# katehai/m-cedm

Hardware: AMD Instinct MI355X
Metric: denoised_states_per_sec_18step_edm_heun (higher is better)
Workload: dtype f32; 1 GPU; SWE-periodic 128x128, EDM U-Net ch=128 ch_mult=[1,1,1,1] attn@16^2 (BASELINE config 3); states_per_gpu=32, global_batch=32, H=128, W=128, sampler=EDM Heun, 18 steps, 35 NFE/state, S_churn=0, w=0, fp64 state / fp32 net, parallelism=batch-sharded x1, no data-path collective, launch=one HIP graph per sampler call

## Files before the change

### m-cedm_amd/csrc/conv_wino.hip

```cpp
#include <atomic>
#include <cstdlib>

#include "conv_wino.hpp"
#include "pack.hpp"
#include "prof.hpp"

namespace mcedm {

__global__ void wino_pack_kernel(const float* __restrict__ w, float* __restrict__ dst, int Cout, int Cin, int coutp, int nch,
                                 int tflip) {
  const int idx = blockIdx.x * blockDim.x + threadIdx.x;
  if (idx >= coutp * nch * WKC) return;
  wino_pack_elem(w, dst, idx, Cout, Cin, coutp, tflip);
}

__global__ void conv_frag_pack_kernel(const float* __restrict__ w, float* __restrict__ dst, int Cout, int Cin, int coutp, int cinp) {
  const int idx = blockIdx.x * blockDim.x + threadIdx.x;
  if (idx >= coutp * cinp) return;
  dst[idx] = frag_pack_value(w, idx, Cout, Cin, coutp);
}

template <class C, bool = C::SKIP>
struct SkipFold {};
template <class C>
struct SkipFold<C, true> {
  static constexpr int SKS = C::SKS, SKBUF = C::SKBUF, SKP = C::SKPITCH;
  __amdgpu_buffer_rsrc_t rs_a, rs_b;
  unsigned voff, HW4;
  int Ca, nsk;
  const f32x4* wf;
  size_t wstride;
  float* wr;
  const float* rd;
  f32x4 sld, sa[2];

  __device__ __forceinline__ f32x4 req(int s) const {
    const int ci0 = SKS * s;
    if (ci0 < Ca) return __builtin_bit_cast(f32x4, __builtin_amdgcn_raw_buffer_load_b128(rs_a, voff, (unsigned)ci0 * HW4, 0));
    return __builtin_bit_cast(f32x4, __builtin_amdgcn_raw_buffer_load_b128(rs_b, voff, (unsigned)(ci0 - Ca) * HW4, 0));
  }
  __device__ __forceinline__ void commit(int buf) const {
    float* d = wr + buf * SKBUF;
    *reinterpret_cast<f32x2*>(d) = f32x2{sld[0], sld[1]};
    *reinterpret_cast<f32x2*>(d + SKP) = f32x2{sld[2], sld[3]};
  }
  __device__ __forceinline__ void wreq(int s, f32x4 (&a)[2]) const {
    a[0] = wf[(size_t)(2 * s) * wstride];
    a[1] = wf[(size_t)(2 * s + 1) * wstride];
  }
  __device__ __forceinline__ void begin(const ConvArgs& p, float* skbuf, int n, int mblk, int mblocks, int y0, int x0, int tid, int lane, int hf) {
    asm volatile("" : "+v"(tid));
    lane = tid & 63;
    const unsigned HW = (unsigned)p.H * (unsigned)p.W;
    HW4 = 4u * HW;
    Ca = p.sk_Ca;
    nsk = (p.sk_Ca + p.sk_Cb) / SKS;
    rs_a = make_rsrc(p.sk_xa + (size_t)n * p.sk_Ca * HW, 4u * (unsigned)p.sk_Ca * HW);
    rs_b = make_rsrc(p.sk_xb ? p.sk_xb + (size_t)n * p.sk_Cb * HW : nullptr, p.sk_xb ? 4u * (unsigned)p.sk_Cb * HW : 0u);
    const int c16 = tid >> 5, row = (tid & 31) >> 2, q = tid & 3;
    voff = 4u * ((unsigned)c16 * HW + (unsigned)(y0 + row) * (unsigned)p.W + (unsigned)(x0 + 4 * q));
    wr = skbuf + ((row & 1) * 32 + (row >> 1) * WTX + 2 * q) * SKP + (c16 & 1) * 16 + 2 * (c16 >> 1);
    rd = skbuf + (hf * 32 + (lane & 31)) * SKP + (lane >> 5) * 16;
    wf = reinterpret_cast<const f32x4*>(p.sk_wfrag) + (size_t)mblk * 64 + lane;
    wstride = (size_t)mblocks * 64;
    sld = req(0);
    wreq(0, sa);
  }
  __device__ __forceinline__ void run(float* xch, const float* skb, int wave, int pw, int lane, const f32x16 (&keep)[2], const f32x16 (&send)[2],
                                      float (&v0)[16], float (&v1)[16]) {
#pragma unroll
    for (int r = 0; r < 16; ++r) xch[(wave * 16 + r) * 64 + lane] = send[0][r];
    commit(0);
    sld = req(1);
    f32x16 rv[2];
    {
      const f32x16 zero16 = {0.f, 0.f, 0.f, 0.f, 0.f, 0.f, 0.f, 0.f, 0.f, 0.f, 0.f, 0.f, 0.f, 0.f, 0.f, 0.f};
      float z = 0.f;
#pragma unroll
      for (int e = 0; e < 2; ++e) {
        asm volatile("" : "+v"(z));
        rv[e] = __builtin_amdgcn_mfma_f32_32x32x2f32(z, z, zero16, 0, 0, 0);
      }
    }
    __syncthreads();
#pragma unroll
    for (int r = 0; r < 16; ++r) v0[r] = keep[0][r] + xch[(pw * 16 + r) * 64 + lane];
    f32x4 bq[4];
#pragma unroll
    for (int jj = 0; jj < 4; ++jj) bq[jj] = *reinterpret_cast<const f32x4*>(rd + 4 * jj);
    for (int s = 0; s < nsk; ++s) {
      f32x4 bqn[4], san[2];
      wreq(s + 1 < nsk ? s + 1 : s, san);
      commit((s + 1) & 1);
      sld = req(s + 2 < nsk ? s + 2 : nsk - 1);
#pragma unroll
      for (int j = 0; j < 4; ++j)
#pragma unroll
        for (int e = 0; e < 2; ++e) rv[e] = __builtin_amdgcn_mfma_f32_32x32x2f32(sa[j >> 2][j & 3], bq[j >> 1][2 * (j & 1) + e], rv[e], 0, 0, 0);
      __syncthreads();
      const float* b = rd + ((s + 1) & 1) * SKBUF;
#pragma unroll
      for (int jj = 0; jj < 4; ++jj) bqn[jj] = *reinterpret_cast<const f32x4*>(b + 4 * jj);
      if (s == 0) {
#pragma unroll
        for (int r = 0; r < 16; ++r) xch[(wave * 16 + r) * 64 + lane] = send[1][r];
      }
      if (s == 1) {
#pragma unroll
        for (int r = 0; r < 16; ++r) v1[r] = keep[1][r] + xch[(pw * 16 + r) * 64 + lane];
      }
#pragma unroll
      for (int j = 4; j < 8; ++j)
#pragma unroll
        for (int e = 0; e < 2; ++e) rv[e] = __builtin_amdgcn_mfma_f32_32x32x2f32(sa[j >> 2][j & 3], bq[j >> 1][2 * (j & 1) + e], rv[e], 0, 0, 0);
#pragma unroll
      for (int jj = 0; jj < 4; ++jj) bq[jj] = bqn[jj];
      sa[0] = san[0];
      sa[1] = san[1];
    }
#pragma unroll
    for (int r = 0; r < 16; ++r) {
      const float bs = skb[(r & 3) + 8 * (r >> 2)];
      v0[r] = v0[r] + (rv[0][r] + bs);
      v1[r] = v1[r] + (rv[1][r] + bs);
    }
  }
};

template <class C, bool UP, bool ACT = true, class... Tag>
__global__ __launch_bounds__(C::NT, C::MB == 4 ? 1 : 2) void conv_wino_kernel(const ConvArgs p, int tiles_x, int tiles_img, int nch, int mblocks,
                                                                          int per, int mode) {
  constexpr int WSC = C::SC, VBUF = C::VBUF, RBUF = C::RBUF, MB = C::MB;
  constexpr bool SKIP = C::SKIP;
  constexpr bool UPZ = WinoUpTraits<Tag...>::UPZ;
  constexpr bool UPS = WinoUpTraits<Tag...>::UPS;
  static_assert(!UPS || UPZ, "source-resolution staging is part of the zero-position variant");
  static_assert(!UPZ || (UP && !SKIP), "the zero positions belong to the up-sampled input");
  constexpr bool SPLIT = C::SPLIT;
  static_assert(!SPLIT || (!UP && !SKIP && sizeof...(Tag) == 0 && MB == 4 && WSC == 2), "the split variant: plain input, WinoCfg<4>'s input path");
  extern __shared__ float lds[];
  const int Cin = p.Ca + p.Cb;
  float* const vbuf = lds;
  float* const rbuf = lds + 2 * VBUF;
  Coef* const cfl = reinterpret_cast<Coef*>(lds + C::LDS_ROWS_OFF);
  float* const xch = lds + C::LDS_ROWS_OFF + 4 * Cin;
  float* const red = xch + C::XCH_FLOATS;
  float* const bias_l = red + 2 * (C::MT / 2) * 3;
  float* const skb_l = bias_l + C::MT;
  float* const skbuf = skb_l + C::MT;
  const int tid = threadIdx.x, lane = tid & 63;
  const int wave = __builtin_amdgcn_readfirstlane(tid >> 6);
  const int mb = wave % MB, hf = wave / MB;
  if (p.dbg && tid == 0) { p.dbg[blockIdx.x * 16 + 0] = __builtin_amdgcn_s_memrealtime(); p.dbg[blockIdx.x * 16 + 4] = per; }
  int gt0 = blockIdx.x * per, tstep = 1;
  int n = gt0 / tiles_img, tile0 = gt0 % tiles_img;
  if (!SPLIT && (mode & 256)) {
    const int nwg = gridDim.x, wps = tiles_img / per;
    const int lid = (nwg % 8 == 0) ? (int)(blockIdx.x % 8) * (nwg / 8) + (int)(blockIdx.x / 8) : (int)blockIdx.x;
    n = lid / wps; tile0 = lid % wps; tstep = wps;
  }
  int split_mb = 0;
  if constexpr (SPLIT) {
    const int nwg = gridDim.x, nmb = p.Cout / C::MT;
    const int lid = (nwg % 8 == 0) ? (int)(blockIdx.x % 8) * (nwg / 8) + (int)(blockIdx.x / 8) : (int)blockIdx.x;
    split_mb = lid % nmb;
    n = (lid / nmb) / tiles_img; tile0 = (lid / nmb) % tiles_img;
  }
  const int m0 = SPLIT ? split_mb * C::MT : blockIdx.y * C::MT;
  const size_t HW = (size_t)p.H * p.W, HWs = (size_t)p.Hs * p.Ws;
  const int nst = (nch + WSC - 1) / WSC;
  const int G = per * nst;

  constexpr int NR = UPS ? 1 : UP ? RSUB : 4, NG = UPS ? 1 : UP ? RSUB : 1;
  unsigned roff[NG], rkeepL[NG], rkeepC[NG];
  int lofs[4];
  if (!UP) {
    const int r = lane / 6, qd = lane % 6;
#pragma unroll
    for (int e = 0; e < 4; ++e) {
      const int col = 4 * qd + e - 3;
      lofs[e] = (lane < 60 && col >= 0 && col < RPITCH) ? r * RPITCH + col : RROWS * RPITCH + lane % (RPLANE - RROWS * RPITCH);
    }
  }
  auto set_geom = [&](int tile) {
    const int y0 = (tile / tiles_x) * WPH, x0 = (tile % tiles_x) * WPW;
    if (UPS) {
      const int r = lane / UCOLS, c = lane - r * UCOLS;
      const int y = (y0 >> 1) - 1 + r, x = (x0 >> 1) - 1 + c;
      const bool inb = lane < UROWS * UCOLS && (unsigned)y < (unsigned)p.Hs && (unsigned)x < (unsigned)p.Ws;
      rkeepL[0] = inb ? 0xffffffffu : 0u;
      roff[0] = !inb ? 0u : 4u * (unsigned)(y * p.Ws + x);
    } else if (UP) {
#pragma unroll
      for (int i = 0; i < NG; ++i) {
        const int e = lane + 64 * i;
        const int r = e / RPITCH, c = e - r * RPITCH;
        const int y = y0 - 1 + r, x = x0 - 1 + c;
        const bool inb = e < RROWS * RPITCH && (unsigned)y < (unsigned)p.H && (unsigned)x < (unsigned)p.W;
        rkeepL[i] = inb ? 0xffffffffu : 0u;
        roff[i] = !inb ? 0u : 4u * (unsigned)((y >> 1) * p.Ws + (x >> 1));
      }
    } else {
      const int y = y0 - 1 + lane / 6, x = x0 - 4 + 4 * (lane % 6);
      const bool inb = lane < 60 && (unsigned)y < (unsigned)p.H && x >= 0 && x < p.W;
      rkeepL[0] = inb ? 0xffffffffu : 0u;
      roff[0] = inb ? 4u * (unsigned)(y * p.W + x) : 0u;
    }
  };
  float raw[WSC][C::CPW][NR];
  int ld_st = 0, ld_tile = tile0, cm_st = 0;
  set_geom(tile0);
  auto raw_load1 = [&](int sc) {
#pragma unroll
    for (int cw = 0; cw < C::CPW; ++cw) {
      const int ci = (ld_st * WSC + sc) * WKC + wave * C::CPW + cw;
      const bool in_a = ci < p.Ca;
      const float* src = in_a ? p.xa : p.xb;
      const int cc = in_a ? ci : ci - p.Ca, CC = in_a ? p.Ca : p.Cb;
      const bool ok = ci < Cin && src != nullptr;
      const float* plane = ok ? src + ((size_t)n * CC + cc) * HWs : (p.xa ? p.xa : p.xb);
      if (UP) {
#pragma unroll
        for (int i = 0; i < NG; ++i) raw[sc][cw][i] = *reinterpret_cast<const float*>(reinterpret_cast<const char*>(plane) + roff[i]);
      } else {
        const f32x4 q = *reinterpret_cast<const f32x4*>(reinterpret_cast<const char*>(plane) + roff[0]);
#pragma unroll
        for (int e = 0; e < 4; ++e) raw[sc][cw][e] = q[e];
      }
    }
  };
  auto raw_load_next = [&]() { if (++ld_st == nst) { ld_st = 0; ld_tile += tstep; set_geom(ld_tile < tiles_img ? ld_tile : tiles_img - 1); } };
  auto raw_load_done = [&]() {
#pragma unroll
    for (int i = 0; i < NG; ++i) rkeepC[i] = rkeepL[i];
  };
  auto raw_load = [&]() {
#pragma unroll
    for (int sc = 0; sc < WSC; ++sc) raw_load1(sc);
    raw_load_done();
    raw_load_next();
  };
  auto raw_commit1 = [&](int sc, float* rb) {
#pragma unroll
    for (int cw = 0; cw < C::CPW; ++cw) {
      const int kl = wave * C::CPW + cw, ci = (cm_st * WSC + sc) * WKC + kl;
      const bool ok = ci < Cin && (ci < p.Ca ? p.xa : p.xb) != nullptr;
      const Coef cf = cfl[ci < Cin ? ci : Cin - 1];
      const unsigned ck = ok ? 0xffffffffu : 0u;
      if (UPS) {
        float v = apply_coef(raw[sc][cw][0], cf, p.act);
        v = __builtin_bit_cast(float, __builtin_bit_cast(unsigned, v) & (rkeepC[0] & ck));
        rb[(sc * WKC + kl) * UPLANE + lane] = v;
      } else if (UP) {
#pragma unroll
        for (int i = 0; i < NR; ++i) {
          float v = apply_coef(raw[sc][cw][i], cf, p.act);
          v = __builtin_bit_cast(float, __builtin_bit_cast(unsigned, v) & (rkeepC[i] & ck));
          if (i + 1 < RSUB || lane + 64 * i < RROWS * RPITCH) rb[(sc * WKC + kl) * RPLANE + lane + 64 * i] = v;
        }
      } else {
        const unsigned mk = rkeepC[0] & ck;
        const float scm = __builtin_bit_cast(float, __builtin_bit_cast(unsigned, cf.scale) & mk);
        const float ofm = __builtin_bit_cast(float, __builtin_bit_cast(unsigned, cf.offset) & mk);
        f32x2 t[2];
#pragma unroll
        for (int h = 0; h < 2; ++h) {
          const f32x2 v = {raw[sc][cw][2 * h], raw[sc][cw][2 * h + 1]};
          t[h] = (v - cf.mean) * scm + ofm;
        }
#pragma unroll
        for (int h = 0; h < 2; ++h) { if constexpr (ACT) t[h] = silu_f2(t[h]); }
#pragma unroll
        for (int i = 0; i < 4; ++i) rb[(sc * WKC + kl) * RPLANE + lofs[i]] = t[i >> 1][i & 1];
      }
    }
  };
  auto commit_done = [&]() { if (++cm_st == nst) cm_st = 0; };
  const int tk = lane & 7, ttx = lane >> 3, tty = mb;
  const int tr_yz = tk * RPLANE + (2 * tty + 2 * hf) * RPITCH + 2 * ttx;
  const int tr_x = tk * RPLANE + (2 * tty + 2 - hf) * RPITCH + 2 * ttx;
  const float tsgn = hf ? -1.f : 1.f;
  const f32x2 tpm = {1.f, -1.f};
  const int tr_dst = (8 * hf) * VPOS + (tk & 1) * VH1 + (tty * WTX + ttx) * 4 + (tk >> 1);
  f32x2 td[WSC][C::TI][3][2];
  const int us_yz = tk * UPLANE + (tty + hf) * UCOLS + ttx, us_x = tk * UPLANE + (tty + 1) * UCOLS + ttx;
  float tu[WSC][C::TI][3][3];
  auto transform_read1 = [&](int sc, const float* rb) {
    if constexpr (UPS) {
#pragma unroll
      for (int ti = 0; ti < C::TI; ++ti) {
        const float* b = rb + sc * WKC * UPLANE + MB * ti * UCOLS;
#pragma unroll
        for (int c = 0; c < 3; ++c) {
          tu[sc][ti][0][c] = b[us_yz + c];
          tu[sc][ti][1][c] = b[us_yz + UCOLS + c];
          tu[sc][ti][2][c] = b[us_x + c];
        }
      }
      return;
    }
#pragma unroll
    for (int ti = 0; ti < C::TI; ++ti)
#pragma unroll
      for (int j = 0; j < 2; ++j) {
        const float* b = rb + sc * WKC * RPLANE + 2 * MB * ti * RPITCH + 2 * j;
        td[sc][ti][0][j] = *reinterpret_cast<const f32x2*>(b + tr_yz);
        td[sc][ti][1][j] = *reinterpret_cast<const f32x2*>(b + tr_yz + RPITCH);
        td[sc][ti][2][j] = *reinterpret_cast<const f32x2*>(b + tr_x);
      }
  };
  auto transform_finish1 = [&](int sc, float* vb) {
    if constexpr (UPS) {
#pragma unroll
      for (int ti = 0; ti < C::TI; ++ti) {
        float t[2][3];
#pragma unroll
        for (int c = 0; c < 3; ++c) {
          t[0][c] = tu[sc][ti][0][c] - tu[sc][ti][2][c];
          t[1][c] = tu[sc][ti][2][c] + tsgn * tu[sc][ti][1][c];
        }
#pragma unroll
        for (int x = 0; x < 2; ++x) {
          if (x == 0 && hf != 0) continue;
          float* o = vb + sc * 16 * VPOS + tr_dst + MB * ti * WTX * 4 + 4 * x * VPOS;
          o[0 * VPOS] = t[x][0] - t[x][1];
          o[1 * VPOS] = t[x][1] + 1.f * t[x][1];
          o[3 * VPOS] = t[x][1] - t[x][2];
        }
      }
      return;
    }
#pragma unroll
    for (int ti = 0; ti < C::TI; ++ti) {
      f32x2 t[2][2];
#pragma unroll
      for (int j = 0; j < 2; ++j) {
        t[0][j] = td[sc][ti][0][j] - td[sc][ti][2][j];
        t[1][j] = td[sc][ti][2][j] + tsgn * td[sc][ti][1][j];
      }
#pragma unroll
      for (int x = 0; x < 2; ++x) {
        const f32x2 o03 = t[x][0] - t[x][1];
        const f32x2 c11 = {t[x][0].y, t[x][0].y}, c22 = {t[x][1].x, t[x][1].x};
        const f32x2 o12 = c11 + tpm * c22;
        float* o = vb + sc * 16 * VPOS + tr_dst + MB * ti * WTX * 4 + 4 * x * VPOS;
        o[0 * VPOS] = o03.x;
        o[1 * VPOS] = o12.x;
        if constexpr (!UPZ) o[2 * VPOS] = o12.y;
        o[3 * VPOS] = o03.y;
      }
    }
  };
  auto transform_read = [&](const float* rb) { for (int sc = 0; sc < WSC; ++sc) transform_read1(sc, rb); };
  auto transform_finish = [&](float* vb) { for (int sc = 0; sc < WSC; ++sc) transform_finish1(sc, vb); };

  stage_coef_rows<C::NT>(p, n, cfl, tid);
  if (tid < C::MT) bias_l[tid] = p.bias ? p.bias[(WinoUpTraits<Tag...>::BROWS ? n * p.bias_batch : 0) + m0 + tid] : 0.f;
  if constexpr (SKIP) { if (tid < C::MT) skb_l[tid] = p.sk_bias ? p.sk_bias[m0 + tid] : 0.f; }
  raw_load();
  __syncthreads();
  for (int sc = 0; sc < WSC; ++sc) raw_commit1(sc, rbuf);
  commit_done();
  if (G > 1) { raw_load(); for (int sc = 0; sc < WSC; ++sc) raw_commit1(sc, rbuf + RBUF); commit_done(); }
  if (G > 2) raw_load();
  const size_t ustride = (size_t)mblocks * 16 * 64;
  constexpr int PHF = UPZ ? 12 : 8;
  const f32x4* up = reinterpret_cast<const f32x4*>(p.wino) + (SPLIT ? ((size_t)(m0 / 32) * 16 + 2 * wave) : ((size_t)(m0 / 32 + mb) * 16 + PHF * hf)) * 64 + lane;
  f32x4 ua[8];
  f32x4 wa[WSC][2];
  if constexpr (SPLIT) {
#pragma unroll
    for (int sc = 0; sc < WSC; ++sc)
#pragma unroll
      for (int q = 0; q < 2; ++q) wa[sc][q] = up[(size_t)(sc < nch ? sc : 0) * ustride + q * 64];
  } else if constexpr (UPZ) {
    const f32x4 zero4 = {0.f, 0.f, 0.f, 0.f};
    ua[0] = up[0 * 64]; ua[1] = up[1 * 64]; ua[3] = up[3 * 64];
    ua[4] = zero4; ua[5] = zero4; ua[7] = zero4;
    if (hf == 0) { ua[4] = up[4 * 64]; ua[5] = up[5 * 64]; ua[7] = up[7 * 64]; }
  } else {
#pragma unroll
    for (int q = 0; q < 8; ++q) ua[q] = up[q * 64];
  }
  __syncthreads();
  transform_read(rbuf);
  transform_finish(vbuf);
  f32x16 acc[8];
  auto init_acc = [&]() {
    const f32x16 zero16 = {0.f, 0.f, 0.f, 0.f, 0.f, 0.f, 0.f, 0.f, 0.f, 0.f, 0.f, 0.f, 0.f, 0.f, 0.f, 0.f};
    float z = 0.f;
#pragma unroll
    for (int q = 0; q < (SPLIT ? 2 : 8); ++q) {
      asm volatile("" : "+v"(z));
      acc[q] = __builtin_amdgcn_mfma_f32_32x32x2f32(z, z, zero16, 0, 0, 0);
    }
    if constexpr (SPLIT) {
      if (wave == 2) {
#pragma unroll
        for (int r = 0; r < 16; ++r) acc[1][r] = bias_l[4 * (lane >> 5) + (r & 3) + 8 * (r >> 2)];
      }
    } else if (hf == 0) {
#pragma unroll
      for (int r = 0; r < 16; ++r) acc[5][r] = bias_l[32 * mb + 4 * (lane >> 5) + (r & 3) + 8 * (r >> 2)];
    }
  };
  __syncthreads();
  init_acc();

  const int vrd = (SPLIT ? 2 * wave : PHF * hf) * VPOS + (lane >> 5) * VH1 + (lane & 31) * 4;
  if (p.dbg && tid == 0) { p.dbg[blockIdx.x * 16 + 1] = __builtin_amdgcn_s_memrealtime(); p.dbg[blockIdx.x * 16 + 5] = __builtin_amdgcn_s_memtime(); }
#ifdef MCEDM_WINO_TIMELINE
  unsigned long long ph[5] = {0, 0, 0, 0, 0}, tlast = __builtin_amdgcn_s_memtime();
#define WINO_STAMP(i) { const unsigned long long t_ = __builtin_amdgcn_s_memtime(); ph[i] += t_ - tlast; tlast = t_; }
  unsigned long long sl[8] = {0, 0, 0, 0, 0, 0, 0, 0}, slast = 0;
#define WINO_SLOT(i) { const unsigned long long t_ = __builtin_amdgcn_s_memtime(); sl[(i) & 7] += t_ - slast; slast = t_; }
#define WINO_SLOT0 { slast = __builtin_amdgcn_s_memtime(); }
  unsigned long long ep[6] = {0, 0, 0, 0, 0, 0}, elast = 0;
#define WINO_EP(i) { __builtin_amdgcn_sched_barrier(0); const unsigned long long t_ = __builtin_amdgcn_s_memtime(); if (i) ep[(i) - 1] += t_ - elast; elast = t_; __builtin_amdgcn_sched_barrier(0); }
  const bool no_u = mode & 2;
#else
#define WINO_STAMP(i)
#define WINO_SLOT(i)
#define WINO_SLOT0
#define WINO_EP(i)
  constexpr bool no_u = false;
#endif
  auto side_slice_upz = [&](int slot, int cur) {
    if (WSC == 2) {
      if (slot == 0) transform_read1(0, rbuf + (cur ^ 1) * RBUF);
      if (slot == 1) raw_commit1(0, rbuf + cur * RBUF);
      if (slot == 2) { transform_finish1(0, vbuf + (cur ^ 1) * VBUF); raw_load1(0); }
      if (slot == 3) transform_read1(WSC - 1, rbuf + (cur ^ 1) * RBUF);
      if (slot == 4) { raw_commit1(WSC - 1, rbuf + cur * RBUF); commit_done(); }
      if (slot == 5) { transform_finish1(WSC - 1, vbuf + (cur ^ 1) * VBUF); raw_load1(WSC - 1); raw_load_done(); }
    } else {
      if (slot == 0) transform_read(rbuf + (cur ^ 1) * RBUF);
      if (slot == 1) { raw_commit1(0, rbuf + cur * RBUF); commit_done(); }
      if (slot == 2) { transform_finish1(0, vbuf + (cur ^ 1) * VBUF); raw_load1(0); raw_load_done(); }
    }
  };
  auto side_slice = [&](int slot, int g, int cur) {
    if (WSC == 2) {
      if (slot == 0) transform_read1(0, rbuf + (cur ^ 1) * RBUF);
      if (slot == 1) raw_commit1(0, rbuf + cur * RBUF);
      if (slot == 2) { transform_finish1(0, vbuf + (cur ^ 1) * VBUF); raw_load1(0); }
      if (slot == 3) transform_read1(WSC - 1, rbuf + (cur ^ 1) * RBUF);
      if (slot == 4) { raw_commit1(WSC - 1, rbuf + cur * RBUF); commit_done(); }
      if (slot == 5) { transform_finish1(WSC - 1, vbuf + (cur ^ 1) * VBUF); raw_load1(WSC - 1); raw_load_done(); }
    } else {
      if (slot == 0) transform_read(rbuf + (cur ^ 1) * RBUF);
      if (slot == 1) { raw_commit1(0, rbuf + cur * RBUF); commit_done(); }
      if (slot == 2) { raw_load1(0); raw_load_done(); }
      if (slot == 3) transform_finish1(0, vbuf + (cur ^ 1) * VBUF);
    }
  };
  (void)mode;
  int st = 0, tile = tile0;
  for (int g = 0; g < G; ++g) {
    const int cur = g & 1;
    WINO_STAMP(0)
    WINO_SLOT0
    if constexpr (SPLIT) {
      f32x4 bf[WSC][2], wn[WSC][2];
#pragma unroll
      for (int sc = 0; sc < WSC; ++sc) {
        const float* vb = vbuf + cur * VBUF + sc * 16 * VPOS + vrd;
        bf[sc][0] = *reinterpret_cast<const f32x4*>(vb);
        bf[sc][1] = *reinterpret_cast<const f32x4*>(vb + VPOS);
      }
#pragma unroll
      for (int sc = 0; sc < WSC; ++sc) {
        const int cn = (st + 1) * WSC + sc;
        const f32x4* un = up + (size_t)(cn < nch ? cn : 0) * ustride;
        wn[sc][0] = un[0];
        wn[sc][1] = un[64];
      }
      __builtin_amdgcn_sched_barrier(0);
#pragma unroll
      for (int sc = 0; sc < WSC; ++sc) {
#pragma unroll
        for (int s = 0; s < 4; ++s) {
          acc[0] = __builtin_amdgcn_mfma_f32_32x32x2f32(wa[sc][0][s], bf[sc][0][s], acc[0], 0, 0, 0);
          acc[1] = __builtin_amdgcn_mfma_f32_32x32x2f32(wa[sc][1][s], bf[sc][1][s], acc[1], 0, 0, 0);
          side_slice(sc * 4 + s, g, cur);
#pragma unroll
          for (int i = 0; i < 2; ++i) {
            __builtin_amdgcn_sched_group_barrier(0x008, 1, 0);
            __builtin_amdgcn_sched_group_barrier(0x486, 4 * WINO_IL_K, 0);
          }
          __builtin_amdgcn_sched_group_barrier(0x020, 4, 0);
          __builtin_amdgcn_sched_barrier(0);
          if (sc * 4 + s == 5) raw_load_next();
          __builtin_amdgcn_sched_barrier(0);
        }
      }
#pragma unroll
      for (int sc = 0; sc < WSC; ++sc) { wa[sc][0] = wn[sc][0]; wa[sc][1] = wn[sc][1]; }
    } else {
#pragma unroll
    for (int sc = 0; sc < WSC; ++sc) {
      const int c = st * WSC + sc;
      const f32x4* un = up + (size_t)(c + 1 < nch ? c + 1 : 0) * ustride;
      const float* vb = vbuf + cur * VBUF + sc * 16 * VPOS + vrd;
      if constexpr (UPZ) {
        constexpr int CQ[3] = {0, 1, 3};
        f32x4 bq[3];
        bq[0] = *reinterpret_cast<const f32x4*>(vb);
        bq[1] = *reinterpret_cast<const f32x4*>(vb + VPOS);
        __builtin_amdgcn_sched_group_barrier(0x100, 2, 0);
#pragma unroll
        for (int i = 0; i < 3; ++i) {
          if (i == 0) bq[2] = *reinterpret_cast<const f32x4*>(vb + 3 * VPOS);
#pragma unroll
          for (int s = 0; s < 4; ++s) acc[CQ[i]] = __builtin_amdgcn_mfma_f32_32x32x2f32(ua[CQ[i]][s], bq[i][s], acc[CQ[i]], 0, 0, 0);
          if (!no_u) ua[CQ[i]] = un[CQ[i] * 64];
          side_slice_upz(sc * 3 + i, cur);
          if (i == 0) __builtin_amdgcn_sched_group_barrier(0x100, 1, 0);
#pragma unroll
          for (int k = 0; k < 4; ++k) {
            __builtin_amdgcn_sched_group_barrier(0x008, 1, 0);
            __builtin_amdgcn_sched_group_barrier(0x486, 2 * WINO_IL_K, 0);
          }
          __builtin_amdgcn_sched_group_barrier(0x020, 4, 0);
          __builtin_amdgcn_sched_barrier(0);
          if (sc * 3 + i == (WSC == 2 ? 5 : 2)) raw_load_next();
          __builtin_amdgcn_sched_barrier(0);
        }
        if (hf == 0) {
          constexpr int HQ[3] = {4, 5, 7};
          f32x4 bh[3];
#pragma unroll
          for (int i = 0; i < 3; ++i) bh[i] = *reinterpret_cast<const f32x4*>(vb + HQ[i] * VPOS);
#pragma unroll
          for (int i = 0; i < 3; ++i) {
#pragma unroll
            for (int s = 0; s < 4; ++s) acc[HQ[i]] = __builtin_amdgcn_mfma_f32_32x32x2f32(ua[HQ[i]][s], bh[i][s], acc[HQ[i]], 0, 0, 0);
            if (!no_u) ua[HQ[i]] = un[HQ[i] * 64];
          }
        }
        __builtin_amdgcn_sched_barrier(0);
      } else {
      f32x4 b4[2][2];
      b4[0][0] = *reinterpret_cast<const f32x4*>(vb);
      b4[0][1] = *reinterpret_cast<const f32x4*>(vb + VPOS);
      __builtin_amdgcn_sched_group_barrier(0x100, 2, 0);
#pragma unroll
      for (int qp = 0; qp < 4; ++qp) {
        const int cb = qp & 1;
        if (qp < 3) {
          b4[cb ^ 1][0] = *reinterpret_cast<const f32x4*>(vb + (2 * qp + 2) * VPOS);
          b4[cb ^ 1][1] = *reinterpret_cast<const f32x4*>(vb + (2 * qp + 3) * VPOS);
        }
#pragma unroll
        for (int s = 0; s < 4; ++s) {
          acc[2 * qp] = __builtin_amdgcn_mfma_f32_32x32x2f32(ua[2 * qp][s], b4[cb][0][s], acc[2 * qp], 0, 0, 0);
          acc[2 * qp + 1] = __builtin_amdgcn_mfma_f32_32x32x2f32(ua[2 * qp + 1][s], b4[cb][1][s], acc[2 * qp + 1], 0, 0, 0);
        }
        if (!no_u) {
          ua[2 * qp] = un[(2 * qp) * 64];
          ua[2 * qp + 1] = un[(2 * qp + 1) * 64];
        }
        side_slice(sc * 4 + qp, g, cur);
        if (qp < 3) __builtin_amdgcn_sched_group_barrier(0x100, 2, 0);
#pragma unroll
        for (int i = 0; i < 8; ++i) {
          __builtin_amdgcn_sched_group_barrier(0x008, 1, 0);
          __builtin_amdgcn_sched_group_barrier(0x486, WINO_IL_K, 0);
        }
        __builtin_amdgcn_sched_group_barrier(0x020, 4, 0);
        __builtin_amdgcn_sched_barrier(0);
        if (sc * 4 + qp == (WSC == 2 ? 5 : 2)) raw_load_next();
        __builtin_amdgcn_sched_barrier(0);
        WINO_SLOT(sc * 4 + qp + (WSC == 1 ? 0 : 0))
      }
      }
    }
    }
    WINO_STAMP(1)
    __syncthreads();
    WINO_STAMP(2)
    if (++st < nst) continue;
    st = 0;

    if constexpr (SPLIT) {
      const int y0 = (tile / tiles_x) * WPH, x0 = (tile % tiles_x) * WPW;
      float* const dump = lds;
#pragma unroll
      for (int q = 0; q < 2; ++q)
#pragma unroll
        for (int r = 0; r < 16; ++r) dump[((2 * wave + q) * 16 + r) * 64 + lane] = acc[q][r];
      const int ehf = wave >> 2, gq = wave & 3, pt = lane & 31;
      const int oy = y0 + 2 * (pt >> 3) + ehf, ox = x0 + 2 * (pt & 7);
      const int cbase = m0 + 8 * gq + 4 * (lane >> 5);
      const size_t splane = (size_t)p.Cout * HW;
      const __amdgpu_buffer_rsrc_t rs_out = make_rsrc(p.out + (size_t)n * splane, 4u * (unsigned)splane);
      const size_t rplane = p.res_mode == RS_DOWN ? splane << 2 : splane;
      const __amdgpu_buffer_rsrc_t rs_res = make_rsrc(p.res ? p.res + (size_t)n * rplane : nullptr, p.res ? 4u * (unsigned)rplane : 0u);
      const unsigned HWu = (unsigned)HW;
      const unsigned voff = 4u * ((unsigned)cbase * HWu + (unsigned)oy * p.W + ox);
      float2 rv[4];
      if (p.res && p.res_mode == RS_DOWN) {
        const unsigned dvoff = 4u * ((unsigned)cbase * (HWu << 2) + (unsigned)(2 * oy) * (unsigned)(2 * p.W) + (unsigned)(2 * ox));
        f32x4 ta[4], tb[4];
#pragma unroll
        for (int k = 0; k < 4; ++k) {
          const unsigned so = 4u * (unsigned)k * (HWu << 2);
          ta[k] = __builtin_bit_cast(f32x4, __builtin_amdgcn_raw_buffer_load_b128(rs_res, dvoff, so, 0));
          tb[k] = __builtin_bit_cast(f32x4, __builtin_amdgcn_raw_buffer_load_b128(rs_res, dvoff + 8u * (unsigned)p.W, so, 0));
        }
#pragma unroll
        for (int k = 0; k < 4; ++k)
          rv[k] = make_float2(0.25f * ((ta[k][0] + ta[k][1]) + (tb[k][0] + tb[k][1])), 0.25f * ((ta[k][2] + ta[k][3]) + (tb[k][2] + tb[k][3])));
      } else {
#pragma unroll
        for (int k = 0; k < 4; ++k) rv[k] = __builtin_bit_cast(float2, __builtin_amdgcn_raw_buffer_load_b64(rs_res, voff, 4u * (unsigned)k * HWu, 0));
      }
      __syncthreads();
      float v0[4], v1[4];
#pragma unroll
      for (int k = 0; k < 4; ++k) {
        float T[3][2];
#pragma unroll
        for (int i = 0; i < 3; ++i) {
          const float* d = dump + ((4 * (ehf + i)) * 16 + 4 * gq + k) * 64 + lane;
          const float a0 = d[0 * 16 * 64], a1 = d[1 * 16 * 64], a2 = d[2 * 16 * 64], a3 = d[3 * 16 * 64];
          T[i][0] = a0 + a1 + a2;
          T[i][1] = a1 - a2 - a3;
        }
        if (ehf == 0) {
          v0[k] = (T[0][0] + T[1][0]) + T[2][0] + rv[k].x;
          v1[k] = (T[0][1] + T[1][1]) + T[2][1] + rv[k].y;
        } else {
          v0[k] = (-T[1][0] - T[2][0]) + T[0][0] + rv[k].x;
          v1[k] = (-T[1][1] - T[2][1]) + T[0][1] + rv[k].y;
        }
      }
#pragma unroll
      for (int k = 0; k < 4; ++k)
        __builtin_amdgcn_raw_buffer_store_b64(__builtin_bit_cast(__attribute__((ext_vector_type(2))) unsigned, make_float2(v0[k], v1[k])), rs_out, voff,
                                              4u * (unsigned)k * HWu, 0);
      if (p.gsum) {
        const bool pairs = p.gsum_rc == 2;
        float a[2], b[2];
#pragma unroll
        for (int e = 0; e < 2; ++e) a[e] = half_sum32((v0[2 * e] + v1[2 * e]) + (v0[2 * e + 1] + v1[2 * e + 1]));
        const float cnt = pairs ? 128.f : 256.f;
        const float mean0 = pairs ? a[0] * (1.0f / 128.0f) : (a[0] + a[1]) * (1.0f / 256.0f);
        const float mean1 = pairs ? a[1] * (1.0f / 128.0f) : mean0;
#pragma unroll
        for (int e = 0; e < 2; ++e) {
          const float mean = e ? mean1 : mean0;
          float q = 0.f;
#pragma unroll
          for (int r = 2 * e; r < 2 * e + 2; ++r) { const float d0 = v0[r] - mean, d1 = v1[r] - mean; q = fmaf(d0, d0, q); q = fmaf(d1, d1, q); }
          b[e] = half_sum32(q);
        }
        if ((lane & 31) == 0) {
          const int quad = 2 * gq + (lane >> 5);
          if (pairs) {
#pragma unroll
            for (int e = 0; e < 2; ++e) {
              float* slot = red + (ehf * (C::MT / 2) + 2 * quad + e) * 3;
              slot[0] = cnt; slot[1] = a[e]; slot[2] = b[e];
            }
          } else {
            float* slot = red + (ehf * (C::MT / 4) + quad) * 3;
            slot[0] = cnt; slot[1] = a[0] + a[1]; slot[2] = b[0] + b[1];
          }
        }
        __syncthreads();
        conv_stats_store<C, 2>(p, red, n, m0, tile, tiles_img, tid);
      }
      break;
    }
    WINO_EP(0)
    const int y0 = (tile / tiles_x) * WPH, x0 = (tile % tiles_x) * WPW;
    const int pt = lane & 31;
    const int oy = y0 + 2 * (pt >> 3) + hf, ox = x0 + 2 * (pt & 7);
    const int cbase = m0 + 32 * mb + 4 * (lane >> 5);
    const size_t splane = (size_t)p.Cout * HW;
    const __amdgpu_buffer_rsrc_t rs_out = make_rsrc(p.out + (size_t)n * splane, 4u * (unsigned)splane);
    const size_t rplane = p.res_mode == RS_UP ? splane >> 2 : p.res_mode == RS_DOWN ? splane << 2 : splane;
    const __amdgpu_buffer_rsrc_t rs_res = make_rsrc(p.res ? p.res + (size_t)n * rplane : nullptr, p.res ? 4u * (unsigned)rplane : 0u);
    const unsigned HWu = (unsigned)HW;
    const unsigned voff = 4u * ((unsigned)cbase * HWu + (unsigned)oy * p.W + ox);
    const unsigned rvoff = 4u * ((unsigned)cbase * (HWu >> 2) + (unsigned)(oy >> 1) * (p.W >> 1) + (ox >> 1));
    f32x16 keep[2], send[2];
    float v0[16], v1[16];
    SkipFold<C> sk;
    if constexpr (SKIP) sk.begin(p, skbuf, n, m0 / 32 + mb, mblocks, y0, x0, tid, lane, hf);
#pragma unroll
    for (int j = 0; j < 2; ++j) {
      const f32x16 t0 = j == 0 ? acc[0] + acc[1] + acc[2] : acc[1] - acc[2] - acc[3];
      const f32x16 t1 = j == 0 ? acc[4] + acc[5] + acc[6] : acc[5] - acc[6] - acc[7];
      if (hf == 0)  { keep[j] = t0 + t1; send[j] = t1; }
      else if (UPZ) { keep[j] = -t1 - t0; send[j] = t1; }
      else          { keep[j] = -t0 - t1; send[j] = t0; }
      __builtin_amdgcn_sched_barrier(0);
    }
    __builtin_amdgcn_sched_barrier(0);
    if constexpr (SKIP) {
      WINO_EP(1)
      sk.run(xch, skb_l + 32 * mb + 4 * (lane >> 5), wave, wave ^ MB, lane, keep, send, v0, v1);
      WINO_EP(2)
    } else {
    float2 rv[16];
    if (p.res && p.res_mode == RS_DOWN) {
      const unsigned dvoff = 4u * ((unsigned)cbase * (HWu << 2) + (unsigned)(2 * oy) * (unsigned)(2 * p.W) + (unsigned)(2 * ox));
#pragma unroll
      for (int r0 = 0; r0 < 16; r0 += 4) {
        f32x4 ta[4], tb[4];
#pragma unroll
        for (int k = 0; k < 4; ++k) {
          const unsigned so = 4u * (unsigned)(((r0 + k) & 3) + 8 * ((r0 + k) >> 2)) * (HWu << 2);
          ta[k] = __builtin_bit_cast(f32x4, __builtin_amdgcn_raw_buffer_load_b128(rs_res, dvoff, so, 0));
          tb[k] = __builtin_bit_cast(f32x4, __builtin_amdgcn_raw_buffer_load_b128(rs_res, dvoff + 8u * (unsigned)p.W, so, 0));
        }
#pragma unroll
        for (int k = 0; k < 4; ++k)
          rv[r0 + k] = make_float2(0.25f * ((ta[k][0] + ta[k][1]) + (tb[k][0] + tb[k][1])), 0.25f * ((ta[k][2] + ta[k][3]) + (tb[k][2] + tb[k][3])));
      }
    } else {
#pragma unroll
      for (int r = 0; r < 16; ++r) {
        const int dr = (r & 3) + 8 * (r >> 2);
        if (p.res && p.res_mode == RS_UP) {
          const float q = __builtin_bit_cast(float, __builtin_amdgcn_raw_buffer_load_b32(rs_res, rvoff, 4u * (unsigned)dr * (HWu >> 2), 0));
          rv[r] = make_float2(q, q);
        } else {
          rv[r] = __builtin_bit_cast(float2, __builtin_amdgcn_raw_buffer_load_b64(rs_res, voff, 4u * (unsigned)dr * HWu, 0));
        }
      }
    }
    WINO_EP(1)
    const int pw = wave ^ MB;
#pragma unroll
    for (int j = 0; j < 2; ++j) {
#pragma unroll
      for (int r = 0; r < 16; ++r) xch[(wave * 16 + r) * 64 + lane] = send[j][r];
      __syncthreads();
#pragma unroll
      for (int r = 0; r < 16; ++r) {
        const float got = xch[(pw * 16 + r) * 64 + lane];
        if (j == 0) v0[r] = keep[0][r] + got + rv[r].x;
        else        v1[r] = keep[1][r] + got + rv[r].y;
      }
      if (j == 0) __syncthreads();
    }
    WINO_EP(2)
    }
#pragma unroll
    for (int r = 0; r < 16; ++r)
      __builtin_amdgcn_raw_buffer_store_b64(__builtin_bit_cast(__attribute__((ext_vector_type(2))) unsigned, make_float2(v0[r], v1[r])), rs_out, voff,
                                            4u * (unsigned)((r & 3) + 8 * (r >> 2)) * HWu, 0);
    WINO_EP(3)
    if (p.gsum) {
      const bool pairs = p.gsum_rc == 2;
#pragma unroll
      for (int gq = 0; gq < 4; ++gq) {
        float a[2], b[2];
#pragma unroll
        for (int e = 0; e < 2; ++e) {
          a[e] = half_sum32((v0[4 * gq + 2 * e] + v1[4 * gq + 2 * e]) + (v0[4 * gq + 2 * e + 1] + v1[4 * gq + 2 * e + 1]));
        }
        const float cnt = pairs ? 128.f : 256.f;
        const float mean0 = pairs ? a[0] * (1.0f / 128.0f) : (a[0] + a[1]) * (1.0f / 256.0f);
        const float mean1 = pairs ? a[1] * (1.0f / 128.0f) : mean0;
#pragma unroll
        for (int e = 0; e < 2; ++e) {
          const float mean = e ? mean1 : mean0;
          float q = 0.f;
#pragma unroll
          for (int r = 4 * gq + 2 * e; r < 4 * gq + 2 * e + 2; ++r) { const float d0 = v0[r] - mean, d1 = v1[r] - mean; q = fmaf(d0, d0, q); q = fmaf(d1, d1, q); }
          b[e] = half_sum32(q);
        }
        if ((lane & 31) == 0) {
          const int quad = 8 * mb + 2 * gq + (lane >> 5);
          if (pairs) {
#pragma unroll
            for (int e = 0; e < 2; ++e) {
              float* slot = red + (hf * (C::MT / 2) + 2 * quad + e) * 3;
              slot[0] = cnt; slot[1] = a[e]; slot[2] = b[e];
            }
          } else {
            float* slot = red + (hf * (C::MT / 4) + quad) * 3;
            slot[0] = cnt; slot[1] = a[0] + a[1]; slot[2] = b[0] + b[1];
          }
        }
      }
      __syncthreads();
      conv_stats_store<C, 2>(p, red, n, m0, tile, tiles_img, tid);
    }
    WINO_EP(4)
    __builtin_amdgcn_sched_barrier(0);
    init_acc();
    tile += tstep;
    WINO_EP(5)
    WINO_STAMP(3)
  }
  if (p.dbg && tid == 0) {
    asm volatile("s_waitcnt vmcnt(0)" ::: "memory");
    p.dbg[blockIdx.x * 16 + 2] = __builtin_amdgcn_s_memrealtime(); p.dbg[blockIdx.x * 16 + 6] = __builtin_amdgcn_s_memtime();
    p.dbg[blockIdx.x * 16 + 3] = __builtin_amdgcn_s_memrealtime();
  }
#ifdef MCEDM_WINO_TIMELINE
  if (p.dbg && tid == 0) for (int i = 0; i < 5; ++i) p.dbg[blockIdx.x * 16 + 8 + i] = ph[i];
  if (p.dbg && tid == 0 && (mode & 16)) for (int i = 0; i < 8; ++i) p.dbg[blockIdx.x * 16 + 8 + i] = sl[i];
  if (p.dbg && tid == 0 && (mode & 32)) for (int i = 0; i < 6; ++i) p.dbg[blockIdx.x * 16 + 8 + i] = ep[i];
  if (p.dbg && tid == 64 * MB && !(mode & 48)) { p.dbg[blockIdx.x * 16 + 13] = ph[1]; p.dbg[blockIdx.x * 16 + 14] = ph[2]; p.dbg[blockIdx.x * 16 + 15] = ph[3]; p.dbg[blockIdx.x * 16 + 7] = ph[0]; }
#endif
}

static int wino_mode_env() {
  static const int env =
      (env_int("MCEDM_WINO_MODE", 0) & ~256) | (env_int("MCEDM_WINO_MAP", 1) ? 256 : 0);
  return env;
}

static int wino_min_hw_env() {
  static const int env = env_int("MCEDM_WINO_MIN_HW", 1024);
  return env;
}

size_t conv_frag_packed_floats(int Cout, int Cin) { return (size_t)cout_padded(Cout) * (size_t)ceil_div(Cin, 8) * 8; }

int launch_pack_conv_frag(const float* w, float* dst, int Cout, int Cin, hipStream_t stream) {
  MCEDM_REQUIRE(w && dst && Cout > 0 && Cin > 0, "pack_conv_frag: bad arguments");
  const int coutp = cout_padded(Cout), cinp = ceil_div(Cin, 8) * 8;
  hipLaunchKernelGGL(conv_frag_pack_kernel, dim3(ceil_div(coutp * cinp, 256)), dim3(256), 0, stream, w, dst, Cout, Cin, coutp, cinp);
  MCEDM_LAUNCH_CHECK("conv_frag_pack_kernel");
  return MCEDM_OK;
}

size_t conv_wino_packed_floats(int Cout, int Cin) { return (size_t)16 * cout_padded(Cout) * (size_t)ceil_div(Cin, WKC) * WKC; }

int launch_pack_conv_wino(const float* w, float* dst, int Cout, int Cin, int transpose_flip, hipStream_t stream) {
  MCEDM_REQUIRE(w && dst && Cout > 0 && Cin > 0, "pack_conv_wino: bad arguments");
  const int coutp = cout_padded(Cout), nch = ceil_div(Cin, WKC);
  hipLaunchKernelGGL(wino_pack_kernel, dim3(ceil_div(coutp * nch * WKC, 256)), dim3(256), 0, stream, w, dst, Cout, Cin, coutp, nch,
                     transpose_flip);
  MCEDM_LAUNCH_CHECK("wino_pack_kernel");
  return MCEDM_OK;
}

static bool conv_wino_fold_ok(const ConvArgs& a) {
  const int Csk = a.sk_Ca + a.sk_Cb;
  const unsigned long long HW = (unsigned long long)a.H * a.W;
  return kernel_switch(KV_CONV_WINO_FOLD) != 0 && a.sk_wfrag && a.resample == RS_NONE && !a.res && a.act && a.Cout % 128 == 0 && a.sk_xa && a.sk_Ca > 0 &&
         a.sk_Cb >= 0 && (a.sk_Cb > 0) == (a.sk_xb != nullptr) && a.sk_Ca % 16 == 0 && a.sk_Cb % 16 == 0 && Csk >= 32 && Csk <= 256 &&
         (((size_t)a.sk_xa | (size_t)a.sk_xb | (size_t)a.sk_wfrag) & 15) == 0 && HW * 4ull * (unsigned long long)a.sk_Ca < (1ull << 32) &&
         HW * 4ull * (unsigned long long)a.sk_Cb < (1ull << 32);
}
bool conv_wino_fold_shape_ok(int Cout, int sk_Ca, int sk_Cb, int H, int W) {
  const int Csk = sk_Ca + sk_Cb;
  return kernel_switch(KV_CONV_WINO_FOLD) != 0 && conv_wino_shape_ok(Cout, Cout, H, W) && Cout % 128 == 0 && sk_Ca > 0 && sk_Ca % 16 == 0 && sk_Cb % 16 == 0 &&
         Csk >= 32 && Csk <= 256 && (unsigned long long)H * W * 4ull * (unsigned long long)(sk_Ca > sk_Cb ? sk_Ca : sk_Cb) < (1ull << 32);
}

bool conv_wino_applicable(const ConvArgs& a, int taps) {
  const bool aligned = a.resample != RS_NONE || (((size_t)a.xa | (size_t)a.xb) & 15) == 0;
  return taps == 9 && a.wino && (a.resample == RS_NONE || a.resample == RS_UP) && a.Cout % 64 == 0 && a.H % WPH == 0 && aligned &&
         a.W % WPW == 0 && (a.Ca + a.Cb) % WKC == 0 && a.Ca % WKC == 0 && (!a.sk_wpk || conv_wino_fold_ok(a)) && ((size_t)a.wino & 15) == 0 &&
         (!a.res || a.res_mode == RS_NONE || a.res_mode == RS_UP || a.res_mode == RS_DOWN) && (a.Ca + a.Cb) <= 1024;
}

int wino_tiles_per_wg(long long total, int tiles_img, int slots) {
  int best = 1;
  double best_t = 1e30;
  for (int d = 1; d <= tiles_img; ++d) {
    if (tiles_img % d) continue;
    const long long wgs = total / d;
    const double t = (double)((wgs + slots - 1) / slots) * (d + 0.2);
    if (t < best_t - 1e-9 || (t < best_t + 1e-9 && d > best)) { best_t = t; best = d; }
  }
  return best;
}

template <class C>
static int launch_wino_cfg(const ConvArgs& a, hipStream_t stream) {
  const int tiles_x = a.W / WPW, tiles_img = tiles_x * (a.H / WPH);
  const long long total = (long long)a.B * tiles_img;
  MCEDM_REQUIRE(total > 0 && total <= 0x7fffffffLL, "conv_wino: grid out of range");
  const int Cin = a.Ca + a.Cb, nch = Cin / WKC;
  int sk_floats = 0;
  if constexpr (C::SKIP) sk_floats = C::SK_FLOATS;
  const int lds_bytes = (C::LDS_ROWS_OFF + 4 * Cin + C::XCH_FLOATS + C::RED_FLOATS + sk_floats) * 4;
  MCEDM_REQUIRE(lds_bytes <= 160 * 1024 / (C::MB == 4 ? 1 : 2), "conv_wino: %d input channels exceed the LDS row table", Cin);
  static std::atomic<bool> attr_set[64];
  static std::atomic<int> ncu[64];
  int dev = 0;
  MCEDM_HIP_TRY(hipGetDevice(&dev));
  MCEDM_REQUIRE(dev >= 0 && dev < 64, "device index %d out of range", dev);
  if (!attr_set[dev].load(std::memory_order_acquire)) {
    int n_cu = 0;
    MCEDM_HIP_TRY(hipDeviceGetAttribute(&n_cu, hipDeviceAttributeMultiprocessorCount, dev));
    ncu[dev].store(n_cu > 0 ? n_cu : 256, std::memory_order_release);
    MCEDM_HIP_TRY(hipFuncSetAttribute((const void*)conv_wino_kernel<C, false>, hipFuncAttributeMaxDynamicSharedMemorySize, 160 * 1024));
    if constexpr (!C::SKIP) {
      MCEDM_HIP_TRY(hipFuncSetAttribute((const void*)conv_wino_kernel<C, true>, hipFuncAttributeMaxDynamicSharedMemorySize, 160 * 1024));
      MCEDM_HIP_TRY(hipFuncSetAttribute((const void*)conv_wino_kernel<C, true, true, WinoUp<true>>, hipFuncAttributeMaxDynamicSharedMemorySize, 160 * 1024));
      MCEDM_HIP_TRY(hipFuncSetAttribute((const void*)conv_wino_kernel<C, true, true, WinoUp<false>>, hipFuncAttributeMaxDynamicSharedMemorySize, 160 * 1024));
      MCEDM_HIP_TRY(hipFuncSetAttribute((const void*)conv_wino_kernel<C, false, false>, hipFuncAttributeMaxDynamicSharedMemorySize, 160 * 1024));
      MCEDM_HIP_TRY(hipFuncSetAttribute((const void*)conv_wino_kernel<C, false, true, WinoBiasRows>, hipFuncAttributeMaxDynamicSharedMemorySize, 160 * 1024));
    }
    attr_set[dev].store(true, std::memory_order_release);
  }
  const int per_env = wino_per_env();
  int per = wino_tiles_per_wg(total, tiles_img, ncu[dev].load(std::memory_order_acquire) * (C::MB == 4 ? 1 : 2));
  if (per_env > 0 && tiles_img % per_env == 0) per = per_env;
  char name[64] = "";
  const bool noact = a.resample != RS_UP && !a.act;
  MCEDM_REQUIRE(a.bias_batch == 0 || (!C::SKIP && a.resample == RS_NONE && a.act && a.bias),
                "conv_wino: a bias row per sample (bias_batch=%d) goes with an un-resampled, activated conv without a folded projection", a.bias_batch);
  const int upz = !C::SKIP && a.resample == RS_UP ? kernel_switch(KV_CONV_WINO_UPZ) : 0;
  if (prof_enabled()) snprintf(name, sizeof(name), "conv_wino_kernel<Wino%sCfg<%d>, %s, %s%s>", C::SKIP ? "Skip" : "", C::MB, a.resample == RS_UP ? "true" : "false",
                               noact ? "false" : "true", a.bias_batch ? ", WinoBiasRows" : upz == 2 ? ", WinoUp<false>" : upz ? ", WinoUp<true>" : "");
  const double px = (double)a.B * a.H * a.W;
  const double skc = C::SKIP ? (double)(a.sk_Ca + a.sk_Cb) : 0.0;
  ProfScope ps(name, 2.0 * px * a.Cout * ((double)Cin * 9 + skc),
               4.0 * ((double)a.B * Cin * a.Hs * a.Ws + px * (a.Cout * (a.res ? 2 : 1) + skc) + (double)a.Cout * (Cin * 9 + skc)), stream);
  if constexpr (C::SKIP)
    hipLaunchKernelGGL((conv_wino_kernel<C, false>), dim3((unsigned)(total / per), a.Cout / C::MT), dim3(C::NT), lds_bytes, stream, a, tiles_x,
                       tiles_img, nch, cout_padded(a.Cout) / 32, per, wino_mode_env());
  else if (a.bias_batch)
    hipLaunchKernelGGL((conv_wino_kernel<C, false, true, WinoBiasRows>), dim3((unsigned)(total / per), a.Cout / C::MT), dim3(C::NT), lds_bytes, stream, a, tiles_x,
                       tiles_img, nch, cout_padded(a.Cout) / 32, per, wino_mode_env());
  else if (upz == 2)
    hipLaunchKernelGGL((conv_wino_kernel<C, true, true, WinoUp<false>>), dim3((unsigned)(total / per), a.Cout / C::MT), dim3(C::NT), lds_bytes, stream, a, tiles_x,
                       tiles_img, nch, cout_padded(a.Cout) / 32, per, wino_mode_env());
  else if (upz)
    hipLaunchKernelGGL((conv_wino_kernel<C, true, true, WinoUp<true>>), dim3((unsigned)(total / per), a.Cout / C::MT), dim3(C::NT), lds_bytes, stream, a, tiles_x,
                       tiles_img, nch, cout_padded(a.Cout) / 32, per, wino_mode_env());
  else if (a.resample == RS_UP)
    hipLaunchKernelGGL((conv_wino_kernel<C, true>), dim3((unsigned)(total / per), a.Cout / C::MT), dim3(C::NT), lds_bytes, stream, a, tiles_x,
                       tiles_img, nch, cout_padded(a.Cout) / 32, per, wino_mode_env());
  else if (noact)
    hipLaunchKernelGGL((conv_wino_kernel<C, false, false>), dim3((unsigned)(total / per), a.Cout / C::MT), dim3(C::NT), lds_bytes, stream, a, tiles_x,
                       tiles_img, nch, cout_padded(a.Cout) / 32, per, wino_mode_env());
  else
    hipLaunchKernelGGL((conv_wino_kernel<C, false>), dim3((unsigned)(total / per), a.Cout / C::MT), dim3(C::NT), lds_bytes, stream, a, tiles_x,
                       tiles_img, nch, cout_padded(a.Cout) / 32, per, wino_mode_env());
  MCEDM_LAUNCH_CHECK("conv_wino_kernel");
  if (a.gsum_tiles) *a.gsum_tiles = SumTiles{tiles_img, tiles_x, WPH, WPW, a.gsum_rc == 2 ? 2 : 4};
  return MCEDM_OK;
}

int launch_conv_wino(const ConvArgs& a_in, hipStream_t stream) {
  ConvArgs a = a_in;
  a.dbg = conv_debug_buffer();
  MCEDM_REQUIRE(conv_wino_applicable(a, 9), "conv_wino: shape not served by the Winograd kernel");
  MCEDM_REQUIRE(a.out && a.B > 0 && (a.resample == RS_UP ? (a.Hs * 2 == a.H && a.Ws * 2 == a.W) : (a.Hs == a.H && a.Ws == a.W)),
                "conv_wino: bad arguments");
  MCEDM_REQUIRE((unsigned long long)a.H * a.W * 4ull * a.Cout * (a.res && a.res_mode == RS_DOWN ? 4 : 1) < (1ull << 32),
                "conv_wino: one sample of the output / residual exceeds the 4 GiB buffer range");
  { const int rc = conv_resolve_identity(a); if (rc != MCEDM_OK) return rc; }
  if (a.sk_wpk) return launch_wino_cfg<WinoSkipCfg<4>>(a, stream);
  if (a.Cout % 128 == 0 && !a.bias_batch) {
    const int rc = try_launch_conv_wino1(a, stream);
    if (rc != -1) return rc;
  }
  return a.Cout % 128 == 0 ? launch_wino_cfg<WinoCfg<4>>(a, stream) : launch_wino_cfg<WinoCfg<2>>(a, stream);
}

bool conv_wino_shape_ok(int Cout, int Cin, int H, int W) {
  return kernel_switch(KV_CONV_WINO) != 0 && Cout % 64 == 0 && Cin % WKC == 0 && H % WPH == 0 && W % WPW == 0 && (long long)H * W >= wino_min_hw_env();
}
bool conv_wino_preferred(const ConvArgs& a) { return kernel_switch(KV_CONV_WINO) != 0 && (long long)a.H * a.W >= wino_min_hw_env(); }

bool conv_wino_small(int H, int W) { return (long long)H * W < wino_min_hw_env(); }
bool conv_wino_split_preferred() { return kernel_switch(KV_CONV_WINO) != 0 && kernel_switch(KV_CONV_WINO_SPLIT) != 0; }
bool conv_wino_split_applicable(const ConvArgs& a, int taps) {
  const int Cin = a.Ca + a.Cb;
  return taps == 9 && a.wino && a.resample == RS_NONE && !a.sk_wpk && a.bias_batch == 0 && conv_wino_small(a.H, a.W) && a.Cout % 32 == 0 &&
         a.H % WPH == 0 && a.W % WPW == 0 && a.Ca > 0 && a.Cb >= 0 && Cin % WKC == 0 && a.Ca % WKC == 0 && Cin <= 1024 &&
         (((size_t)a.xa | (size_t)a.xb | (size_t)a.wino) & 15) == 0 && (!a.res || a.res_mode == RS_NONE || a.res_mode == RS_DOWN);
}

int launch_conv_wino_split(const ConvArgs& a_in, hipStream_t stream) {
  typedef WinoSplitCfg C;
  ConvArgs a = a_in;
  a.dbg = nullptr;
  MCEDM_REQUIRE(conv_wino_split_applicable(a, 9), "conv_wino_split: shape not served by the split Winograd kernel");
  MCEDM_REQUIRE(a.out && a.B > 0 && a.Hs == a.H && a.Ws == a.W, "conv_wino_split: bad arguments");
  MCEDM_REQUIRE((unsigned long long)a.H * a.W * 4ull * a.Cout * (a.res && a.res_mode == RS_DOWN ? 4 : 1) < (1ull << 32),
                "conv_wino_split: one sample of the output / residual exceeds the 4 GiB buffer range");
  { const int rc = conv_resolve_identity(a); if (rc != MCEDM_OK) return rc; }
  const int tiles_x = a.W / WPW, tiles_img = tiles_x * (a.H / WPH), nmb = a.Cout / C::MT;
  const long long total = (long long)a.B * tiles_img * nmb;
  MCEDM_REQUIRE(total > 0 && total <= 0x7fffffffLL, "conv_wino_split: grid out of range");
  const int Cin = a.Ca + a.Cb, nch = Cin / WKC;
  const int lds_bytes = (C::LDS_ROWS_OFF + 4 * Cin + C::XCH_FLOATS + C::RED_FLOATS) * 4;
  MCEDM_REQUIRE(lds_bytes <= 160 * 1024, "conv_wino_split: %d input channels exceed the LDS row table", Cin);
  static std::atomic<bool> attr_set[64];
  int dev = 0;
  MCEDM_HIP_TRY(hipGetDevice(&dev));
  MCEDM_REQUIRE(dev >= 0 && dev < 64, "device index %d out of range", dev);
  if (!attr_set[dev].load(std::memory_order_acquire)) {
    MCEDM_HIP_TRY(hipFuncSetAttribute((const void*)conv_wino_kernel<C, false>, hipFuncAttributeMaxDynamicSharedMemorySize, 160 * 1024));
    MCEDM_HIP_TRY(hipFuncSetAttribute((const void*)conv_wino_kernel<C, false, false>, hipFuncAttributeMaxDynamicSharedMemorySize, 160 * 1024));
    attr_set[dev].store(true, std::memory_order_release);
  }
  char name[64] = "";
  if (prof_enabled()) snprintf(name, sizeof(name), "conv_wino_kernel<WinoSplitCfg, false, %s>", a.act ? "true" : "false");
  const double px = (double)a.B * a.H * a.W;
  ProfScope ps(name, 2.0 * px * a.Cout * (double)Cin * 9,
               4.0 * ((double)a.B * Cin * a.H * a.W + px * a.Cout * (a.res ? 2 : 1) + (double)a.Cout * Cin * 9), stream);
  if (a.act)
    hipLaunchKernelGGL((conv_wino_kernel<C, false>), dim3((unsigned)total), dim3(C::NT), lds_bytes, stream, a, tiles_x, tiles_img, nch,
                       cout_padded(a.Cout) / 32, 1, 0);
  else
    hipLaunchKernelGGL((conv_wino_kernel<C, false, false>), dim3((unsigned)total), dim3(C::NT), lds_bytes, stream, a, tiles_x, tiles_img, nch,
                       cout_padded(a.Cout) / 32, 1, 0);
  MCEDM_LAUNCH_CHECK("conv_wino_kernel");
  if (a.gsum_tiles) *a.gsum_tiles = SumTiles{tiles_img, tiles_x, WPH, WPW, a.gsum_rc == 2 ? 2 : 4};
  return MCEDM_OK;
}

}
```

### m-cedm_amd/csrc/conv_wino.hpp

```cpp
#pragma once
#include "conv_tile.hpp"

namespace mcedm {

constexpr int WPH = 8, WPW = 16;
constexpr int WTX = WPW / 2, WTY = WPH / 2;
constexpr int WKC = 8;
static_assert(WTX * WTY == 32, "one MFMA N block of patches per workgroup");
template <int MB_>
struct WinoCfg {
  static constexpr int MB = MB_, NT = 128 * MB_, NW = 2 * MB_, MT = 32 * MB_;
  static constexpr int SC = MB_ == 4 ? 2 : 1;
  static constexpr int CPW = WKC / NW;
  static constexpr int TI = 4 / MB_;
  static constexpr int VBUF = SC * 16 * 288, RBUF = SC * WKC * 196;
  static constexpr int LDS_ROWS_OFF = 2 * VBUF + 2 * RBUF;
  static constexpr int XCH_FLOATS = NW * 16 * 64;
  static constexpr int RED_FLOATS = 2 * (MT / 2) * 3 + MT;
  static constexpr bool SKIP = false;
  static constexpr bool SPLIT = false;
  static_assert(MB_ == 4 || MB_ == 2, "128 or 64 output channels per workgroup");
  static_assert(LDS_ROWS_OFF % 4 == 0, "LDS layout");
};
struct WinoSplitCfg : WinoCfg<4> {
  static constexpr int MT = 32;
  static constexpr int XCH_FLOATS = 0;
  static constexpr int RED_FLOATS = 2 * (MT / 2) * 3 + MT;
  static constexpr int DUMP_FLOATS = 16 * 16 * 64;
  static constexpr bool SPLIT = true;
  static_assert(DUMP_FLOATS <= 2 * VBUF, "the accumulator dump fits the two V buffers");
};
template <int MB_>
struct WinoSkipCfg : WinoCfg<MB_> {
  static constexpr bool SKIP = true;
  static constexpr int SKS = 16, SKPITCH = 36, SKBUF = 64 * SKPITCH;
  static constexpr int SK_FLOATS = WinoCfg<MB_>::MT + 2 * SKBUF;
  static_assert(MB_ == 4, "the fold is built for the 128-channel workgroup (512 threads = 16 channels x 32 quads per stage)");
};
template <bool SRC>
struct WinoUp {};
template <class... Tag>
struct WinoUpTraits { static constexpr bool UPZ = false, UPS = false, BROWS = false; static_assert(sizeof...(Tag) == 0, "one tag at most: WinoUp<SRC> or WinoBiasRows"); };
template <bool SRC>
struct WinoUpTraits<WinoUp<SRC>> { static constexpr bool UPZ = true, UPS = SRC, BROWS = false; };
struct WinoBiasRows {};
template <>
struct WinoUpTraits<WinoBiasRows> { static constexpr bool UPZ = false, UPS = false, BROWS = true; };
constexpr int UROWS = WPH / 2 + 2, UCOLS = WPW / 2 + 2;
constexpr int UPLANE = 68;
static_assert(UPLANE >= 64 && UPLANE % 32 == 4 && UPLANE <= 196, "LDS layout");
constexpr int RROWS = WPH + 2, RPITCH = WPW + 2;
constexpr int RPLANE = 196;
constexpr int RSUB = (RROWS * RPITCH + 63) / 64;
constexpr int WINO_IL_K = 5;
constexpr int VH1 = 144, VPOS = 288;
static_assert(RPLANE % 32 == 4 && VH1 % 32 == 16 && VH1 >= 128 && VPOS >= VH1 + 128 && RPLANE >= RROWS * RPITCH && RPLANE % 2 == 0 && VPOS % 4 == 0 && VH1 % 4 == 0, "LDS layout");



int try_launch_conv_wino1(const ConvArgs& a, hipStream_t stream);
int wino_tiles_per_wg(long long total, int tiles_img, int slots);
inline int wino_per_env() { static const int v = env_int("MCEDM_WINO_PER", 0); return v; }

}
```

Before: 83.23 states/s.

## Use LDS base-plus-immediate addressing, packed f32 transforms, and buffer-load weight fragments

Replaces pointer-based LDS accesses in the Winograd conv kernel with per-lane LDS byte addresses that take compile-time immediate offsets, so each access needs fewer address VALU ops and fewer live registers. The input-transform arithmetic now uses explicit v_pk_add/v_pk_fma instructions. Weight fragments are fetched through buffer loads with a scalar chunk offset in a new 'pair' form. A WinoLoop1 template variant keeps the old global-pointer weight loads and is chosen at launch time, which doubles kernel instantiations. Static asserts check that offsets fit the 16-bit immediate field.

After: 88.79 states/s, median of 6. +6.7%, better.

```diff
diff --git a/m-cedm_amd/csrc/conv_wino.hip b/m-cedm_amd/csrc/conv_wino.hip
--- a/m-cedm_amd/csrc/conv_wino.hip
+++ b/m-cedm_amd/csrc/conv_wino.hip
@@ -127,6 +127,31 @@
   }
 };
 
+template <class T>
+__device__ __forceinline__ T lds_get(unsigned base, int off) {
+  return *reinterpret_cast<const __attribute__((address_space(3))) T*>(base + (unsigned)off);
+}
+template <class T>
+__device__ __forceinline__ void lds_put(unsigned base, int off, T v) {
+  *reinterpret_cast<__attribute__((address_space(3))) T*>(base + (unsigned)off) = v;
+}
+__device__ __forceinline__ f32x2 pk_sub(f32x2 a, f32x2 b) {
+  f32x2 d;
+  asm("v_pk_add_f32 %0, %1, %2 neg_lo:[0,1] neg_hi:[0,1]" : "=v"(d) : "v"(a), "v"(b));
+  return d;
+}
+__device__ __forceinline__ f32x2 pk_fma(f32x2 a, f32x2 b, f32x2 c) {
+  f32x2 d;
+  asm("v_pk_fma_f32 %0, %1, %2, %3" : "=v"(d) : "v"(a), "v"(b), "v"(c));
+  return d;
+}
+__device__ __forceinline__ f32x2 pk_hi_pm_lo(f32x2 a, f32x2 b) {
+  f32x2 d;
+  asm("v_pk_add_f32 %0, %1, %2 op_sel:[1,0] op_sel_hi:[1,0] neg_hi:[0,1]" : "=v"(d) : "v"(a), "v"(b));
+  return d;
+}
+#define WINO_LDS_IMM_OK(floats, bytes) static_assert(4 * (floats) + (bytes) <= 65536, "LDS offset beyond the 16-bit immediate field")
+
 template <class C, bool UP, bool ACT = true, class... Tag>
 __global__ __launch_bounds__(C::NT, C::MB == 4 ? 1 : 2) void conv_wino_kernel(const ConvArgs p, int tiles_x, int tiles_img, int nch, int mblocks,
                                                                           int per, int mode) {
@@ -134,14 +159,13 @@
   constexpr bool SKIP = C::SKIP;
   constexpr bool UPZ = WinoUpTraits<Tag...>::UPZ;
   constexpr bool UPS = WinoUpTraits<Tag...>::UPS;
+  constexpr bool PAIR = !WinoUpTraits<Tag...>::LOOP1;
   static_assert(!UPS || UPZ, "source-resolution staging is part of the zero-position variant");
   static_assert(!UPZ || (UP && !SKIP), "the zero positions belong to the up-sampled input");
   constexpr bool SPLIT = C::SPLIT;
-  static_assert(!SPLIT || (!UP && !SKIP && sizeof...(Tag) == 0 && MB == 4 && WSC == 2), "the split variant: plain input, WinoCfg<4>'s input path");
+  static_assert(!SPLIT || (!UP && !SKIP && !UPZ && !WinoUpTraits<Tag...>::BROWS && MB == 4 && WSC == 2), "the split variant: plain input, WinoCfg<4>'s input path");
   extern __shared__ float lds[];
   const int Cin = p.Ca + p.Cb;
-  float* const vbuf = lds;
-  float* const rbuf = lds + 2 * VBUF;
   Coef* const cfl = reinterpret_cast<Coef*>(lds + C::LDS_ROWS_OFF);
   float* const xch = lds + C::LDS_ROWS_OFF + 4 * Cin;
   float* const red = xch + C::XCH_FLOATS;
@@ -151,6 +175,8 @@
   const int tid = threadIdx.x, lane = tid & 63;
   const int wave = __builtin_amdgcn_readfirstlane(tid >> 6);
   const int mb = wave % MB, hf = wave / MB;
+  const unsigned lds0 = (unsigned)reinterpret_cast<size_t>((__attribute__((address_space(3))) float*)lds);
+  constexpr int RB0 = 4 * 2 * VBUF;
   if (p.dbg && tid == 0) { p.dbg[blockIdx.x * 16 + 0] = __builtin_amdgcn_s_memrealtime(); p.dbg[blockIdx.x * 16 + 4] = per; }
   int gt0 = blockIdx.x * per, tstep = 1;
   int n = gt0 / tiles_img, tile0 = gt0 % tiles_img;
@@ -173,15 +199,22 @@
 
   constexpr int NR = UPS ? 1 : UP ? RSUB : 4, NG = UPS ? 1 : UP ? RSUB : 1;
   unsigned roff[NG], rkeepL[NG], rkeepC[NG];
-  int lofs[4];
+  constexpr int NCM = UP ? 1 : 4;
+  unsigned cm_a[NCM];
   if (!UP) {
     const int r = lane / 6, qd = lane % 6;
 #pragma unroll
     for (int e = 0; e < 4; ++e) {
       const int col = 4 * qd + e - 3;
-      lofs[e] = (lane < 60 && col >= 0 && col < RPITCH) ? r * RPITCH + col : RROWS * RPITCH + lane % (RPLANE - RROWS * RPITCH);
-    }
-  }
+      const int lofs = (lane < 60 && col >= 0 && col < RPITCH) ? r * RPITCH + col : RROWS * RPITCH + lane % (RPLANE - RROWS * RPITCH);
+      cm_a[e] = lds0 + RB0 + 4 * (wave * C::CPW * RPLANE + lofs);
+    }
+  } else {
+    cm_a[0] = lds0 + RB0 + 4 * (wave * C::CPW * (UPS ? UPLANE : RPLANE) + lane);
+  }
+#pragma unroll
+  for (int e = 0; e < NCM; ++e) asm volatile("" : "+v"(cm_a[e]));
+  WINO_LDS_IMM_OK(RBUF + ((WSC - 1) * WKC + C::CPW - 1) * RPLANE + (UP && !UPS ? 64 * (RSUB - 1) : 0), 4);
   auto set_geom = [&](int tile) {
     const int y0 = (tile / tiles_x) * WPH, x0 = (tile % tiles_x) * WPW;
     if (UPS) {
@@ -240,7 +273,7 @@
     raw_load_done();
     raw_load_next();
   };
-  auto raw_commit1 = [&](int sc, float* rb) {
+  auto raw_commit1 = [&](int sc, int rbo) {
 #pragma unroll
     for (int cw = 0; cw < C::CPW; ++cw) {
       const int kl = wave * C::CPW + cw, ci = (cm_st * WSC + sc) * WKC + kl;
@@ -250,13 +283,13 @@
       if (UPS) {
         float v = apply_coef(raw[sc][cw][0], cf, p.act);
         v = __builtin_bit_cast(float, __builtin_bit_cast(unsigned, v) & (rkeepC[0] & ck));
-        rb[(sc * WKC + kl) * UPLANE + lane] = v;
+        lds_put(cm_a[0], rbo + 4 * (sc * WKC + cw) * UPLANE, v);
       } else if (UP) {
 #pragma unroll
         for (int i = 0; i < NR; ++i) {
           float v = apply_coef(raw[sc][cw][i], cf, p.act);
           v = __builtin_bit_cast(float, __builtin_bit_cast(unsigned, v) & (rkeepC[i] & ck));
-          if (i + 1 < RSUB || lane + 64 * i < RROWS * RPITCH) rb[(sc * WKC + kl) * RPLANE + lane + 64 * i] = v;
+          if (i + 1 < RSUB || lane + 64 * i < RROWS * RPITCH) lds_put(cm_a[0], rbo + 4 * ((sc * WKC + cw) * RPLANE + 64 * i), v);
         }
       } else {
         const unsigned mk = rkeepC[0] & ck;
@@ -271,30 +304,32 @@
 #pragma unroll
         for (int h = 0; h < 2; ++h) { if constexpr (ACT) t[h] = silu_f2(t[h]); }
 #pragma unroll
-        for (int i = 0; i < 4; ++i) rb[(sc * WKC + kl) * RPLANE + lofs[i]] = t[i >> 1][i & 1];
+        for (int i = 0; i < 4; ++i) lds_put(cm_a[UP ? 0 : i], rbo + 4 * (sc * WKC + cw) * RPLANE, (float)t[i >> 1][i & 1]);
       }
     }
   };
   auto commit_done = [&]() { if (++cm_st == nst) cm_st = 0; };
   const int tk = lane & 7, ttx = lane >> 3, tty = mb;
-  const int tr_yz = tk * RPLANE + (2 * tty + 2 * hf) * RPITCH + 2 * ttx;
-  const int tr_x = tk * RPLANE + (2 * tty + 2 - hf) * RPITCH + 2 * ttx;
+  unsigned tr_yz = lds0 + RB0 + 4 * (UPS ? tk * UPLANE + (tty + hf) * UCOLS + ttx : tk * RPLANE + (2 * tty + 2 * hf) * RPITCH + 2 * ttx);
+  unsigned tr_x = lds0 + RB0 + 4 * (UPS ? tk * UPLANE + (tty + 1) * UCOLS + ttx : tk * RPLANE + (2 * tty + 2 - hf) * RPITCH + 2 * ttx);
   const float tsgn = hf ? -1.f : 1.f;
-  const f32x2 tpm = {1.f, -1.f};
-  const int tr_dst = (8 * hf) * VPOS + (tk & 1) * VH1 + (tty * WTX + ttx) * 4 + (tk >> 1);
+  const f32x2 tsgn2 = {tsgn, tsgn};
+  unsigned tr_dst = lds0 + 4 * ((8 * hf) * VPOS + (tk & 1) * VH1 + (tty * WTX + ttx) * 4 + (tk >> 1));
+  asm volatile("" : "+v"(tr_yz), "+v"(tr_x), "+v"(tr_dst));
+  WINO_LDS_IMM_OK(RBUF + (WSC - 1) * WKC * (UPS ? UPLANE : RPLANE) + (C::TI - 1) * MB * (UPS ? UCOLS : 2 * RPITCH) + (UPS ? UCOLS + 2 : RPITCH + 2), UPS ? 4 : 8);
+  WINO_LDS_IMM_OK(VBUF + (WSC - 1) * 16 * VPOS + (C::TI - 1) * MB * WTX * 4 + 7 * VPOS, 4);
   f32x2 td[WSC][C::TI][3][2];
-  const int us_yz = tk * UPLANE + (tty + hf) * UCOLS + ttx, us_x = tk * UPLANE + (tty + 1) * UCOLS + ttx;
   float tu[WSC][C::TI][3][3];
-  auto transform_read1 = [&](int sc, const float* rb) {
+  auto transform_read1 = [&](int sc, int rbo) {
     if constexpr (UPS) {
 #pragma unroll
       for (int ti = 0; ti < C::TI; ++ti) {
-        const float* b = rb + sc * WKC * UPLANE + MB * ti * UCOLS;
+        const int b = rbo + 4 * (sc * WKC * UPLANE + MB * ti * UCOLS);
 #pragma unroll
         for (int c = 0; c < 3; ++c) {
-          tu[sc][ti][0][c] = b[us_yz + c];
-          tu[sc][ti][1][c] = b[us_yz + UCOLS + c];
-          tu[sc][ti][2][c] = b[us_x + c];
+          tu[sc][ti][0][c] = lds_get<float>(tr_yz, b + 4 * c);
+          tu[sc][ti][1][c] = lds_get<float>(tr_yz, b + 4 * (UCOLS + c));
+          tu[sc][ti][2][c] = lds_get<float>(tr_x, b + 4 * c);
         }
       }
       return;
@@ -303,13 +338,13 @@
     for (int ti = 0; ti < C::TI; ++ti)
 #pragma unroll
       for (int j = 0; j < 2; ++j) {
-        const float* b = rb + sc * WKC * RPLANE + 2 * MB * ti * RPITCH + 2 * j;
-        td[sc][ti][0][j] = *reinterpret_cast<const f32x2*>(b + tr_yz);
-        td[sc][ti][1][j] = *reinterpret_cast<const f32x2*>(b + tr_yz + RPITCH);
-        td[sc][ti][2][j] = *reinterpret_cast<const f32x2*>(b + tr_x);
+        const int b = rbo + 4 * (sc * WKC * RPLANE + 2 * MB * ti * RPITCH + 2 * j);
+        td[sc][ti][0][j] = lds_get<f32x2>(tr_yz, b);
+        td[sc][ti][1][j] = lds_get<f32x2>(tr_yz, b + 4 * RPITCH);
+        td[sc][ti][2][j] = lds_get<f32x2>(tr_x, b);
       }
   };
-  auto transform_finish1 = [&](int sc, float* vb) {
+  auto transform_finish1 = [&](int sc, int vbo) {
     if constexpr (UPS) {
 #pragma unroll
       for (int ti = 0; ti < C::TI; ++ti) {
@@ -322,10 +357,10 @@
 #pragma unroll
         for (int x = 0; x < 2; ++x) {
           if (x == 0 && hf != 0) continue;
-          float* o = vb + sc * 16 * VPOS + tr_dst + MB * ti * WTX * 4 + 4 * x * VPOS;
-          o[0 * VPOS] = t[x][0] - t[x][1];
-          o[1 * VPOS] = t[x][1] + 1.f * t[x][1];
-          o[3 * VPOS] = t[x][1] - t[x][2];
+          const int o = vbo + 4 * (sc * 16 * VPOS + MB * ti * WTX * 4 + 4 * x * VPOS);
+          lds_put(tr_dst, o + 4 * 0 * VPOS, t[x][0] - t[x][1]);
+          lds_put(tr_dst, o + 4 * 1 * VPOS, t[x][1] + 1.f * t[x][1]);
+          lds_put(tr_dst, o + 4 * 3 * VPOS, t[x][1] - t[x][2]);
         }
       }
       return;
@@ -335,56 +370,68 @@
       f32x2 t[2][2];
 #pragma unroll
       for (int j = 0; j < 2; ++j) {
-        t[0][j] = td[sc][ti][0][j] - td[sc][ti][2][j];
-        t[1][j] = td[sc][ti][2][j] + tsgn * td[sc][ti][1][j];
+        t[0][j] = pk_sub(td[sc][ti][0][j], td[sc][ti][2][j]);
+        t[1][j] = pk_fma(tsgn2, td[sc][ti][1][j], td[sc][ti][2][j]);
       }
 #pragma unroll
       for (int x = 0; x < 2; ++x) {
-        const f32x2 o03 = t[x][0] - t[x][1];
-        const f32x2 c11 = {t[x][0].y, t[x][0].y}, c22 = {t[x][1].x, t[x][1].x};
-        const f32x2 o12 = c11 + tpm * c22;
-        float* o = vb + sc * 16 * VPOS + tr_dst + MB * ti * WTX * 4 + 4 * x * VPOS;
-        o[0 * VPOS] = o03.x;
-        o[1 * VPOS] = o12.x;
-        if constexpr (!UPZ) o[2 * VPOS] = o12.y;
-        o[3 * VPOS] = o03.y;
+        const f32x2 o03 = pk_sub(t[x][0], t[x][1]);
+        const f32x2 o12 = pk_hi_pm_lo(t[x][0], t[x][1]);
+        const int o = vbo + 4 * (sc * 16 * VPOS + MB * ti * WTX * 4 + 4 * x * VPOS);
+        lds_put(tr_dst, o + 4 * 0 * VPOS, (float)o03.x);
+        lds_put(tr_dst, o + 4 * 1 * VPOS, (float)o12.x);
+        if constexpr (!UPZ) lds_put(tr_dst, o + 4 * 2 * VPOS, (float)o12.y);
+        lds_put(tr_dst, o + 4 * 3 * VPOS, (float)o03.y);
       }
     }
   };
-  auto transform_read = [&](const float* rb) { for (int sc = 0; sc < WSC; ++sc) transform_read1(sc, rb); };
-  auto transform_finish = [&](float* vb) { for (int sc = 0; sc < WSC; ++sc) transform_finish1(sc, vb); };
+  auto transform_read = [&](int rbo) { for (int sc = 0; sc < WSC; ++sc) transform_read1(sc, rbo); };
+  auto transform_finish = [&](int vbo) { for (int sc = 0; sc < WSC; ++sc) transform_finish1(sc, vbo); };
 
   stage_coef_rows<C::NT>(p, n, cfl, tid);
   if (tid < C::MT) bias_l[tid] = p.bias ? p.bias[(WinoUpTraits<Tag...>::BROWS ? n * p.bias_batch : 0) + m0 + tid] : 0.f;
   if constexpr (SKIP) { if (tid < C::MT) skb_l[tid] = p.sk_bias ? p.sk_bias[m0 + tid] : 0.f; }
   raw_load();
   __syncthreads();
-  for (int sc = 0; sc < WSC; ++sc) raw_commit1(sc, rbuf);
+  for (int sc = 0; sc < WSC; ++sc) raw_commit1(sc, 0);
   commit_done();
-  if (G > 1) { raw_load(); for (int sc = 0; sc < WSC; ++sc) raw_commit1(sc, rbuf + RBUF); commit_done(); }
+  if (G > 1) { raw_load(); for (int sc = 0; sc < WSC; ++sc) raw_commit1(sc, 4 * RBUF); commit_done(); }
   if (G > 2) raw_load();
   const size_t ustride = (size_t)mblocks * 16 * 64;
   constexpr int PHF = UPZ ? 12 : 8;
-  const f32x4* up = reinterpret_cast<const f32x4*>(p.wino) + (SPLIT ? ((size_t)(m0 / 32) * 16 + 2 * wave) : ((size_t)(m0 / 32 + mb) * 16 + PHF * hf)) * 64 + lane;
+  const size_t upos = (SPLIT ? ((size_t)(m0 / 32) * 16 + 2 * wave) : ((size_t)(m0 / 32 + mb) * 16 + PHF * hf)) * 64 + lane;
+  const f32x4* up = reinterpret_cast<const f32x4*>(p.wino) + upos;
+  const unsigned ustride_b = 16u * (unsigned)ustride;
+  const __amdgpu_buffer_rsrc_t rs_w = make_rsrc(PAIR ? p.wino : nullptr, PAIR ? (unsigned)nch * ustride_b : 0u);
+  unsigned uw[2] = {16u * (unsigned)upos, 16u * (unsigned)upos + 4096u};
+  if constexpr (PAIR) asm volatile("" : "+v"(uw[0]), "+v"(uw[1]));
+  auto wfrag = [&](int chunk, int q) -> f32x4 {
+    if constexpr (PAIR) {
+      asm("" : "+v"(uw[q >> 2]));
+      return __builtin_bit_cast(f32x4, __builtin_amdgcn_raw_buffer_load_b128(rs_w, uw[q >> 2] + (unsigned)(q & 3) * 1024u, (unsigned)chunk * ustride_b, 0));
+    } else {
+      return up[(size_t)chunk * ustride + q * 64];
+    }
+  };
   f32x4 ua[8];
   f32x4 wa[WSC][2];
   if constexpr (SPLIT) {
 #pragma unroll
     for (int sc = 0; sc < WSC; ++sc)
 #pragma unroll
-      for (int q = 0; q < 2; ++q) wa[sc][q] = up[(size_t)(sc < nch ? sc : 0) * ustride + q * 64];
+      for (int q = 0; q < 2; ++q) wa[sc][q] = wfrag(sc < nch ? sc : 0, q);
   } else if constexpr (UPZ) {
     const f32x4 zero4 = {0.f, 0.f, 0.f, 0.f};
-    ua[0] = up[0 * 64]; ua[1] = up[1 * 64]; ua[3] = up[3 * 64];
+    ua[0] = wfrag(0, 0); ua[1] = wfrag(0, 1); ua[3] = wfrag(0, 3);
     ua[4] = zero4; ua[5] = zero4; ua[7] = zero4;
-    if (hf == 0) { ua[4] = up[4 * 64]; ua[5] = up[5 * 64]; ua[7] = up[7 * 64]; }
+    if (hf == 0) { ua[4] = wfrag(0, 4); ua[5] = wfrag(0, 5); ua[7] = wfrag(0, 7); }
   } else {
 #pragma unroll
-    for (int q = 0; q < 8; ++q) ua[q] = up[q * 64];
+    for (int q = 0; q < 8; ++q) ua[q] = wfrag(0, q);
   }
   __syncthreads();
-  transform_read(rbuf);
-  transform_finish(vbuf);
+  transform_read(0);
+  transform_finish(0);
   f32x16 acc[8];
   auto init_acc = [&]() {
     const f32x16 zero16 = {0.f, 0.f, 0.f, 0.f, 0.f, 0.f, 0.f, 0.f, 0.f, 0.f, 0.f, 0.f, 0.f, 0.f, 0.f, 0.f};
@@ -407,7 +454,9 @@
   __syncthreads();
   init_acc();
 
-  const int vrd = (SPLIT ? 2 * wave : PHF * hf) * VPOS + (lane >> 5) * VH1 + (lane & 31) * 4;
+  unsigned vrd = lds0 + 4 * ((SPLIT ? 2 * wave : PHF * hf) * VPOS + (lane >> 5) * VH1 + (lane & 31) * 4);
+  asm volatile("" : "+v"(vrd));
+  WINO_LDS_IMM_OK(VBUF + (WSC - 1) * 16 * VPOS + 7 * VPOS, 16);
   if (p.dbg && tid == 0) { p.dbg[blockIdx.x * 16 + 1] = __builtin_amdgcn_s_memrealtime(); p.dbg[blockIdx.x * 16 + 5] = __builtin_amdgcn_s_memtime(); }
 #ifdef MCEDM_WINO_TIMELINE
   unsigned long long ph[5] = {0, 0, 0, 0, 0}, tlast = __builtin_amdgcn_s_memtime();
@@ -427,53 +476,54 @@
 #endif
   auto side_slice_upz = [&](int slot, int cur) {
     if (WSC == 2) {
-      if (slot == 0) transform_read1(0, rbuf + (cur ^ 1) * RBUF);
-      if (slot == 1) raw_commit1(0, rbuf + cur * RBUF);
-      if (slot == 2) { transform_finish1(0, vbuf + (cur ^ 1) * VBUF); raw_load1(0); }
-      if (slot == 3) transform_read1(WSC - 1, rbuf + (cur ^ 1) * RBUF);
-      if (slot == 4) { raw_commit1(WSC - 1, rbuf + cur * RBUF); commit_done(); }
-      if (slot == 5) { transform_finish1(WSC - 1, vbuf + (cur ^ 1) * VBUF); raw_load1(WSC - 1); raw_load_done(); }
+      if (slot == 0) transform_read1(0, 4 * (cur ^ 1) * RBUF);
+      if (slot == 1) raw_commit1(0, 4 * cur * RBUF);
+      if (slot == 2) { transform_finish1(0, 4 * (cur ^ 1) * VBUF); raw_load1(0); }
+      if (slot == 3) transform_read1(WSC - 1, 4 * (cur ^ 1) * RBUF);
+      if (slot == 4) { raw_commit1(WSC - 1, 4 * cur * RBUF); commit_done(); }
+      if (slot == 5) { transform_finish1(WSC - 1, 4 * (cur ^ 1) * VBUF); raw_load1(WSC - 1); raw_load_done(); }
     } else {
-      if (slot == 0) transform_read(rbuf + (cur ^ 1) * RBUF);
-      if (slot == 1) { raw_commit1(0, rbuf + cur * RBUF); commit_done(); }
-      if (slot == 2) { transform_finish1(0, vbuf + (cur ^ 1) * VBUF); raw_load1(0); raw_load_done(); }
+      if (slot == 0) transform_read(4 * (cur ^ 1) * RBUF);
+      if (slot == 1) { raw_commit1(0, 4 * cur * RBUF); commit_done(); }
+      if (slot == 2) { transform_finish1(0, 4 * (cur ^ 1) * VBUF); raw_load1(0); raw_load_done(); }
     }
   };
   auto side_slice = [&](int slot, int g, int cur) {
     if (WSC == 2) {
-      if (slot == 0) transform_read1(0, rbuf + (cur ^ 1) * RBUF);
-      if (slot == 1) raw_commit1(0, rbuf + cur * RBUF);
-      if (slot == 2) { transform_finish1(0, vbuf + (cur ^ 1) * VBUF); raw_load1(0); }
-      if (slot == 3) transform_read1(WSC - 1, rbuf + (cur ^ 1) * RBUF);
-      if (slot == 4) { raw_commit1(WSC - 1, rbuf + cur * RBUF); commit_done(); }
-      if (slot == 5) { transform_finish1(WSC - 1, vbuf + (cur ^ 1) * VBUF); raw_load1(WSC - 1); raw_load_done(); }
+      if (slot == 0) transform_read1(0, 4 * (cur ^ 1) * RBUF);
+      if (slot == 1) raw_commit1(0, 4 * cur * RBUF);
+      if (slot == 2) { transform_finish1(0, 4 * (cur ^ 1) * VBUF); raw_load1(0); }
+      if (slot == 3) transform_read1(WSC - 1, 4 * (cur ^ 1) * RBUF);
+      if (slot == 4) { raw_commit1(WSC - 1, 4 * cur * RBUF); commit_done(); }
+      if (slot == 5) { transform_finish1(WSC - 1, 4 * (cur ^ 1) * VBUF); raw_load1(WSC - 1); raw_load_done(); }
     } else {
-      if (slot == 0) transform_read(rbuf + (cur ^ 1) * RBUF);
-      if (slot == 1) { raw_commit1(0, rbuf + cur * RBUF); commit_done(); }
+      if (slot == 0) transform_read(4 * (cur ^ 1) * RBUF);
+      if (slot == 1) { raw_commit1(0, 4 * cur * RBUF); commit_done(); }
       if (slot == 2) { raw_load1(0); raw_load_done(); }
-      if (slot == 3) transform_finish1(0, vbuf + (cur ^ 1) * VBUF);
+      if (slot == 3) transform_finish1(0, 4 * (cur ^ 1) * VBUF);
     }
   };
   (void)mode;
   int st = 0, tile = tile0;
-  for (int g = 0; g < G; ++g) {
-    const int cur = g & 1;
+  for (int g = 0; g < G; g += PAIR ? 2 : 1) {
+#pragma unroll
+    for (int half = 0; half < (PAIR ? 2 : 1); ++half) {
+    const int cur = PAIR ? half : g & 1;
     WINO_STAMP(0)
     WINO_SLOT0
     if constexpr (SPLIT) {
       f32x4 bf[WSC][2], wn[WSC][2];
 #pragma unroll
       for (int sc = 0; sc < WSC; ++sc) {
-        const float* vb = vbuf + cur * VBUF + sc * 16 * VPOS + vrd;
-        bf[sc][0] = *reinterpret_cast<const f32x4*>(vb);
-        bf[sc][1] = *reinterpret_cast<const f32x4*>(vb + VPOS);
+        const int vbo = 4 * (cur * VBUF + sc * 16 * VPOS);
+        bf[sc][0] = lds_get<f32x4>(vrd, vbo);
+        bf[sc][1] = lds_get<f32x4>(vrd, vbo + 4 * VPOS);
       }
 #pragma unroll
       for (int sc = 0; sc < WSC; ++sc) {
         const int cn = (st + 1) * WSC + sc;
-        const f32x4* un = up + (size_t)(cn < nch ? cn : 0) * ustride;
-        wn[sc][0] = un[0];
-        wn[sc][1] = un[64];
+        wn[sc][0] = wfrag(cn < nch ? cn : 0, 0);
+        wn[sc][1] = wfrag(cn < nch ? cn : 0, 1);
       }
       __builtin_amdgcn_sched_barrier(0);
 #pragma unroll
@@ -500,20 +550,20 @@
 #pragma unroll
     for (int sc = 0; sc < WSC; ++sc) {
       const int c = st * WSC + sc;
-      const f32x4* un = up + (size_t)(c + 1 < nch ? c + 1 : 0) * ustride;
-      const float* vb = vbuf + cur * VBUF + sc * 16 * VPOS + vrd;
+      const int cn = c + 1 < nch ? c + 1 : 0;
+      const int vbo = 4 * (cur * VBUF + sc * 16 * VPOS);
       if constexpr (UPZ) {
         constexpr int CQ[3] = {0, 1, 3};
         f32x4 bq[3];
-        bq[0] = *reinterpret_cast<const f32x4*>(vb);
-        bq[1] = *reinterpret_cast<const f32x4*>(vb + VPOS);
+        bq[0] = lds_get<f32x4>(vrd, vbo);
+        bq[1] = lds_get<f32x4>(vrd, vbo + 4 * VPOS);
         __builtin_amdgcn_sched_group_barrier(0x100, 2, 0);
 #pragma unroll
         for (int i = 0; i < 3; ++i) {
-          if (i == 0) bq[2] = *reinterpret_cast<const f32x4*>(vb + 3 * VPOS);
+          if (i == 0) bq[2] = lds_get<f32x4>(vrd, vbo + 4 * 3 * VPOS);
 #pragma unroll
           for (int s = 0; s < 4; ++s) acc[CQ[i]] = __builtin_amdgcn_mfma_f32_32x32x2f32(ua[CQ[i]][s], bq[i][s], acc[CQ[i]], 0, 0, 0);
-          if (!no_u) ua[CQ[i]] = un[CQ[i] * 64];
+          if (!no_u) ua[CQ[i]] = wfrag(cn, CQ[i]);
           side_slice_upz(sc * 3 + i, cur);
           if (i == 0) __builtin_amdgcn_sched_group_barrier(0x100, 1, 0);
 #pragma unroll
@@ -530,26 +580,26 @@
           constexpr int HQ[3] = {4, 5, 7};
           f32x4 bh[3];
 #pragma unroll
-          for (int i = 0; i < 3; ++i) bh[i] = *reinterpret_cast<const f32x4*>(vb + HQ[i] * VPOS);
+          for (int i = 0; i < 3; ++i) bh[i] = lds_get<f32x4>(vrd, vbo + 4 * HQ[i] * VPOS);
 #pragma unroll
           for (int i = 0; i < 3; ++i) {
 #pragma unroll
             for (int s = 0; s < 4; ++s) acc[HQ[i]] = __builtin_amdgcn_mfma_f32_32x32x2f32(ua[HQ[i]][s], bh[i][s], acc[HQ[i]], 0, 0, 0);
-            if (!no_u) ua[HQ[i]] = un[HQ[i] * 64];
+            if (!no_u) ua[HQ[i]] = wfrag(cn, HQ[i]);
           }
         }
         __builtin_amdgcn_sched_barrier(0);
       } else {
       f32x4 b4[2][2];
-      b4[0][0] = *reinterpret_cast<const f32x4*>(vb);
-      b4[0][1] = *reinterpret_cast<const f32x4*>(vb + VPOS);
+      b4[0][0] = lds_get<f32x4>(vrd, vbo);
+      b4[0][1] = lds_get<f32x4>(vrd, vbo + 4 * VPOS);
       __builtin_amdgcn_sched_group_barrier(0x100, 2, 0);
 #pragma unroll
       for (int qp = 0; qp < 4; ++qp) {
         const int cb = qp & 1;
         if (qp < 3) {
-          b4[cb ^ 1][0] = *reinterpret_cast<const f32x4*>(vb + (2 * qp + 2) * VPOS);
-          b4[cb ^ 1][1] = *reinterpret_cast<const f32x4*>(vb + (2 * qp + 3) * VPOS);
+          b4[cb ^ 1][0] = lds_get<f32x4>(vrd, vbo + 4 * (2 * qp + 2) * VPOS);
+          b4[cb ^ 1][1] = lds_get<f32x4>(vrd, vbo + 4 * (2 * qp + 3) * VPOS);
         }
 #pragma unroll
         for (int s = 0; s < 4; ++s) {
@@ -557,8 +607,8 @@
           acc[2 * qp + 1] = __builtin_amdgcn_mfma_f32_32x32x2f32(ua[2 * qp + 1][s], b4[cb][1][s], acc[2 * qp + 1], 0, 0, 0);
         }
         if (!no_u) {
-          ua[2 * qp] = un[(2 * qp) * 64];
-          ua[2 * qp + 1] = un[(2 * qp + 1) * 64];
+          ua[2 * qp] = wfrag(cn, 2 * qp);
+          ua[2 * qp + 1] = wfrag(cn, 2 * qp + 1);
         }
         side_slice(sc * 4 + qp, g, cur);
         if (qp < 3) __builtin_amdgcn_sched_group_barrier(0x100, 2, 0);
@@ -579,7 +629,9 @@
     WINO_STAMP(1)
     __syncthreads();
     WINO_STAMP(2)
-    if (++st < nst) continue;
+    ++st;
+    }
+    if (st < nst) continue;
     st = 0;
 
     if constexpr (SPLIT) {
@@ -874,6 +926,34 @@
     if (t < best_t - 1e-9 || (t < best_t + 1e-9 && d > best)) { best_t = t; best = d; }
   }
   return best;
+}
+
+template <class C, bool UP, bool ACT, class... Tag>
+constexpr bool wino_pair_form = !(UP && sizeof...(Tag) == 0) && !(C::MB == 2 && !UP && !ACT);
+static bool wino_loop1(const ConvArgs& a, int chunks_per_stage) {
+  const unsigned long long Cin = (unsigned long long)(a.Ca + a.Cb);
+  const int nst = ceil_div((int)Cin / WKC, chunks_per_stage);
+  const unsigned long long table = 16ull * Cin * (unsigned long long)cout_padded(a.Cout) * 4ull;
+  return nst % 2 != 0 || table >= (1ull << 32);
+}
+template <class C, bool UP, bool ACT, class... Tag>
+static void wino_launch(bool loop1, dim3 grid, int lds_bytes, hipStream_t stream, const ConvArgs& a, int tiles_x, int tiles_img, int nch, int mblocks, int per,
+                        int mode) {
+  if constexpr (wino_pair_form<C, UP, ACT, Tag...>) {
+    if (!loop1) {
+      hipLaunchKernelGGL((conv_wino_kernel<C, UP, ACT, Tag...>), grid, dim3(C::NT), lds_bytes, stream, a, tiles_x, tiles_img, nch, mblocks, per, mode);
+      return;
+    }
+  }
+  hipLaunchKernelGGL((conv_wino_kernel<C, UP, ACT, WinoLoop1, Tag...>), grid, dim3(C::NT), lds_bytes, stream, a, tiles_x, tiles_img, nch, mblocks, per, mode);
+}
+template <class C, bool UP, bool ACT, class... Tag>
+static hipError_t wino_lds_attr() {
+  if constexpr (wino_pair_form<C, UP, ACT, Tag...>) {
+    const hipError_t e = hipFuncSetAttribute((const void*)conv_wino_kernel<C, UP, ACT, Tag...>, hipFuncAttributeMaxDynamicSharedMemorySize, 160 * 1024);
+    if (e != hipSuccess) return e;
+  }
+  return hipFuncSetAttribute((const void*)conv_wino_kernel<C, UP, ACT, WinoLoop1, Tag...>, hipFuncAttributeMaxDynamicSharedMemorySize, 160 * 1024);
 }
 
 template <class C>
@@ -895,13 +975,13 @@
     int n_cu = 0;
     MCEDM_HIP_TRY(hipDeviceGetAttribute(&n_cu, hipDeviceAttributeMultiprocessorCount, dev));
     ncu[dev].store(n_cu > 0 ? n_cu : 256, std::memory_order_release);
-    MCEDM_HIP_TRY(hipFuncSetAttribute((const void*)conv_wino_kernel<C, false>, hipFuncAttributeMaxDynamicSharedMemorySize, 160 * 1024));
+    MCEDM_HIP_TRY((wino_lds_attr<C, false, true>()));
     if constexpr (!C::SKIP) {
-      MCEDM_HIP_TRY(hipFuncSetAttribute((const void*)conv_wino_kernel<C, true>, hipFuncAttributeMaxDynamicSharedMemorySize, 160 * 1024));
-      MCEDM_HIP_TRY(hipFuncSetAttribute((const void*)conv_wino_kernel<C, true, true, WinoUp<true>>, hipFuncAttributeMaxDynamicSharedMemorySize, 160 * 1024));
-      MCEDM_HIP_TRY(hipFuncSetAttribute((const void*)conv_wino_kernel<C, true, true, WinoUp<false>>, hipFuncAttributeMaxDynamicSharedMemorySize, 160 * 1024));
-      MCEDM_HIP_TRY(hipFuncSetAttribute((const void*)conv_wino_kernel<C, false, false>, hipFuncAttributeMaxDynamicSharedMemorySize, 160 * 1024));
-      MCEDM_HIP_TRY(hipFuncSetAttribute((const void*)conv_wino_kernel<C, false, true, WinoBiasRows>, hipFuncAttributeMaxDynamicSharedMemorySize, 160 * 1024));
+      MCEDM_HIP_TRY((wino_lds_attr<C, true, true>()));
+      MCEDM_HIP_TRY((wino_lds_attr<C, true, true, WinoUp<true>>()));
+      MCEDM_HIP_TRY((wino_lds_attr<C, true, true, WinoUp<false>>()));
+      MCEDM_HIP_TRY((wino_lds_attr<C, false, false>()));
+      MCEDM_HIP_TRY((wino_lds_attr<C, false, true, WinoBiasRows>()));
     }
     attr_set[dev].store(true, std::memory_order_release);
   }
@@ -919,27 +999,23 @@
   const double skc = C::SKIP ? (double)(a.sk_Ca + a.sk_Cb) : 0.0;
   ProfScope ps(name, 2.0 * px * a.Cout * ((double)Cin * 9 + skc),
                4.0 * ((double)a.B * Cin * a.Hs * a.Ws + px * (a.Cout * (a.res ? 2 : 1) + skc) + (double)a.Cout * (Cin * 9 + skc)), stream);
+  const dim3 grid((unsigned)(total / per), a.Cout / C::MT);
+  const int mblocks = cout_padded(a.Cout) / 32, mode = wino_mode_env();
+  const bool loop1 = wino_loop1(a, C::SC);
   if constexpr (C::SKIP)
-    hipLaunchKernelGGL((conv_wino_kernel<C, false>), dim3((unsigned)(total / per), a.Cout / C::MT), dim3(C::NT), lds_bytes, stream, a, tiles_x,
-                       tiles_img, nch, cout_padded(a.Cout) / 32, per, wino_mode_env());
+    wino_launch<C, false, true>(loop1, grid, lds_bytes, stream, a, tiles_x, tiles_img, nch, mblocks, per, mode);
   else if (a.bias_batch)
-    hipLaunchKernelGGL((conv_wino_kernel<C, false, true, WinoBiasRows>), dim3((unsigned)(total / per), a.Cout / C::MT), dim3(C::NT), lds_bytes, stream, a, tiles_x,
-                       tiles_img, nch, cout_padded(a.Cout) / 32, per, wino_mode_env());
+    wino_launch<C, false, true, WinoBiasRows>(loop1, grid, lds_bytes, stream, a, tiles_x, tiles_img, nch, mblocks, per, mode);
   else if (upz == 2)
-    hipLaunchKernelGGL((conv_wino_kernel<C, true, true, WinoUp<false>>), dim3((unsigned)(total / per), a.Cout / C::MT), dim3(C::NT), lds_bytes, stream, a, tiles_x,
-                       tiles_img, nch, cout_padded(a.Cout) / 32, per, wino_mode_env());
+    wino_launch<C, true, true, WinoUp<false>>(loop1, grid, lds_bytes, stream, a, tiles_x, tiles_img, nch, mblocks, per, mode);
   else if (upz)
-    hipLaunchKernelGGL((conv_wino_kernel<C, true, true, WinoUp<true>>), dim3((unsigned)(total / per), a.Cout / C::MT), dim3(C::NT), lds_bytes, stream, a, tiles_x,
-                       tiles_img, nch, cout_padded(a.Cout) / 32, per, wino_mode_env());
+    wino_launch<C, true, true, WinoUp<true>>(loop1, grid, lds_bytes, stream, a, tiles_x, tiles_img, nch, mblocks, per, mode);
   else if (a.resample == RS_UP)
-    hipLaunchKernelGGL((conv_wino_kernel<C, true>), dim3((unsigned)(total / per), a.Cout / C::MT), dim3(C::NT), lds_bytes, stream, a, tiles_x,
-                       tiles_img, nch, cout_padded(a.Cout) / 32, per, wino_mode_env());
+    wino_launch<C, true, true>(loop1, grid, lds_bytes, stream, a, tiles_x, tiles_img, nch, mblocks, per, mode);
   else if (noact)
-    hipLaunchKernelGGL((conv_wino_kernel<C, false, false>), dim3((unsigned)(total / per), a.Cout / C::MT), dim3(C::NT), lds_bytes, stream, a, tiles_x,
-                       tiles_img, nch, cout_padded(a.Cout) / 32, per, wino_mode_env());
+    wino_launch<C, false, false>(loop1, grid, lds_bytes, stream, a, tiles_x, tiles_img, nch, mblocks, per, mode);
   else
-    hipLaunchKernelGGL((conv_wino_kernel<C, false>), dim3((unsigned)(total / per), a.Cout / C::MT), dim3(C::NT), lds_bytes, stream, a, tiles_x,
-                       tiles_img, nch, cout_padded(a.Cout) / 32, per, wino_mode_env());
+    wino_launch<C, false, true>(loop1, grid, lds_bytes, stream, a, tiles_x, tiles_img, nch, mblocks, per, mode);
   MCEDM_LAUNCH_CHECK("conv_wino_kernel");
   if (a.gsum_tiles) *a.gsum_tiles = SumTiles{tiles_img, tiles_x, WPH, WPW, a.gsum_rc == 2 ? 2 : 4};
   return MCEDM_OK;
@@ -996,8 +1072,8 @@
   MCEDM_HIP_TRY(hipGetDevice(&dev));
   MCEDM_REQUIRE(dev >= 0 && dev < 64, "device index %d out of range", dev);
   if (!attr_set[dev].load(std::memory_order_acquire)) {
-    MCEDM_HIP_TRY(hipFuncSetAttribute((const void*)conv_wino_kernel<C, false>, hipFuncAttributeMaxDynamicSharedMemorySize, 160 * 1024));
-    MCEDM_HIP_TRY(hipFuncSetAttribute((const void*)conv_wino_kernel<C, false, false>, hipFuncAttributeMaxDynamicSharedMemorySize, 160 * 1024));
+    MCEDM_HIP_TRY((wino_lds_attr<C, false, true>()));
+    MCEDM_HIP_TRY((wino_lds_attr<C, false, false>()));
     attr_set[dev].store(true, std::memory_order_release);
   }
   char name[64] = "";
@@ -1005,12 +1081,11 @@
   const double px = (double)a.B * a.H * a.W;
   ProfScope ps(name, 2.0 * px * a.Cout * (double)Cin * 9,
                4.0 * ((double)a.B * Cin * a.H * a.W + px * a.Cout * (a.res ? 2 : 1) + (double)a.Cout * Cin * 9), stream);
+  const bool loop1 = wino_loop1(a, C::SC);
   if (a.act)
-    hipLaunchKernelGGL((conv_wino_kernel<C, false>), dim3((unsigned)total), dim3(C::NT), lds_bytes, stream, a, tiles_x, tiles_img, nch,
-                       cout_padded(a.Cout) / 32, 1, 0);
+    wino_launch<C, false, true>(loop1, dim3((unsigned)total), lds_bytes, stream, a, tiles_x, tiles_img, nch, cout_padded(a.Cout) / 32, 1, 0);
   else
-    hipLaunchKernelGGL((conv_wino_kernel<C, false, false>), dim3((unsigned)total), dim3(C::NT), lds_bytes, stream, a, tiles_x, tiles_img, nch,
-                       cout_padded(a.Cout) / 32, 1, 0);
+    wino_launch<C, false, false>(loop1, dim3((unsigned)total), lds_bytes, stream, a, tiles_x, tiles_img, nch, cout_padded(a.Cout) / 32, 1, 0);
   MCEDM_LAUNCH_CHECK("conv_wino_kernel");
   if (a.gsum_tiles) *a.gsum_tiles = SumTiles{tiles_img, tiles_x, WPH, WPW, a.gsum_rc == 2 ? 2 : 4};
   return MCEDM_OK;
diff --git a/m-cedm_amd/csrc/conv_wino.hpp b/m-cedm_amd/csrc/conv_wino.hpp
--- a/m-cedm_amd/csrc/conv_wino.hpp
+++ b/m-cedm_amd/csrc/conv_wino.hpp
@@ -40,12 +40,15 @@
 template <bool SRC>
 struct WinoUp {};
 template <class... Tag>
-struct WinoUpTraits { static constexpr bool UPZ = false, UPS = false, BROWS = false; static_assert(sizeof...(Tag) == 0, "one tag at most: WinoUp<SRC> or WinoBiasRows"); };
+struct WinoUpTraits { static constexpr bool UPZ = false, UPS = false, BROWS = false, LOOP1 = false; static_assert(sizeof...(Tag) == 0, "one tag at most: WinoUp<SRC> or WinoBiasRows"); };
 template <bool SRC>
-struct WinoUpTraits<WinoUp<SRC>> { static constexpr bool UPZ = true, UPS = SRC, BROWS = false; };
+struct WinoUpTraits<WinoUp<SRC>> { static constexpr bool UPZ = true, UPS = SRC, BROWS = false, LOOP1 = false; };
 struct WinoBiasRows {};
 template <>
-struct WinoUpTraits<WinoBiasRows> { static constexpr bool UPZ = false, UPS = false, BROWS = true; };
+struct WinoUpTraits<WinoBiasRows> { static constexpr bool UPZ = false, UPS = false, BROWS = true, LOOP1 = false; };
+struct WinoLoop1 {};
+template <class... Tag>
+struct WinoUpTraits<WinoLoop1, Tag...> : WinoUpTraits<Tag...> { static constexpr bool LOOP1 = true; };
 constexpr int UROWS = WPH / 2 + 2, UCOLS = WPW / 2 + 2;
 constexpr int UPLANE = 68;
 static_assert(UPLANE >= 64 && UPLANE % 32 == 4 && UPLANE <= 196, "LDS layout");
```
